# metarank/metarank

Hardware: AMD Instinct MI355X
Metric: ranked items/sec (feature assembly + 500-tree LambdaMART + ordering), Ranklens-shaped 100-item requests (higher is better)
Workload: dtype f64

## Files before the change

metarank_amd/__init__.py:

```python
from ._native import MrkError, build, lib, reload_switches
from .booster import LIGHTGBM, XGBOOST, Context, HipBooster, default_context
from .index import HipIndex
from .ranker import Batch, HipRanker, Server
from .request import Request, RequestSet
from .trending import HipTrending, TrendingBuilder
from .als import AlsBuilder
from .eval import eval_scores, evaluate, labels_from_interactions
from .train import Trainer, bin_bounds, fit_lambdamart, lambdarank_gradients
```

metarank_amd/_native.py:

```python
from __future__ import annotations

import ctypes as C
import os
import subprocess
import threading

HERE = os.path.dirname(os.path.abspath(__file__))
REPO = os.path.dirname(HERE)
CSRC = os.path.join(HERE, "csrc")
LIB_PATH = os.environ.get("MRK_LIB") or os.path.join(HERE, "libmrk_hip.so")
SOURCES = ["forest.cpp", "store.cpp", "features.cpp", "codec.cpp", "tokenizer.cpp", "weights.cpp", "capi.cpp", "capi_rank.cpp", "capi_encoder.cpp", "comm.cpp", "jit.cpp", "score.hip", "score_qs.hip", "rank.hip", "resolve.hip", "writes.hip", "encoder.hip"]
HEADERS = ["json.hpp", "forest.hpp", "runtime.hpp"]

MRK_OK = 0
ERR_INVALID_ARG, ERR_PARSE, ERR_DEVICE, ERR_DIM_MISMATCH = -1, -2, -3, -4
ERR_ARITHMETIC, ERR_UNSUPPORTED, ERR_NOT_FOUND, ERR_FEATURE_MISMATCH = -5, -6, -7, -8


class MrkError(RuntimeError):
    def __init__(self, status: int, message: str):
        super().__init__(f"[{status}] {message}")
        self.status = status
        self.message = message


def sources():
    extra = sorted(f for f in os.listdir(CSRC) if f.endswith((".cpp", ".hip")) and f not in SOURCES)
    return [os.path.join(CSRC, f) for f in SOURCES + extra]


JIT_HEADERS = ["device_types.hpp", "rank.hpp", "qs_device.hpp", "sort_device.hpp", "table_device.hpp", "walk_device.hpp", "wave_device.hpp", "rank_device.hpp"]


def embed_jit_sources() -> str:
    parts = []
    for h in JIT_HEADERS:
        lines = [ln for ln in open(os.path.join(CSRC, h)).read().split("\n")
                 if not ln.startswith("#include") and not ln.startswith("#pragma once")]
        parts.append(f"// ---- {h}\n" + "\n".join(lines))
    text = "\n".join(parts)
    assert ')MRKJIT"' not in text
    out = "\n".join('R"MRKJIT(' + p + '\n)MRKJIT"' for p in parts) + "\n"
    path = os.path.join(CSRC, "jit_embed.inc")
    if not os.path.exists(path) or open(path).read() != out:
        with open(path, "w") as f:
            f.write(out)
    return path


def write_build_id() -> str:
    import hashlib

    h = hashlib.sha256()
    for f in sorted(os.listdir(CSRC)):
        if f.endswith((".cpp", ".hip", ".hpp")):
            h.update(f.encode() + b"\0" + open(os.path.join(CSRC, f), "rb").read())
    h.update(open(os.path.join(REPO, "include", "mrk.h"), "rb").read())
    out = '"' + h.hexdigest()[:16] + '"\n'
    path = os.path.join(CSRC, "build_id.inc")
    if not os.path.exists(path) or open(path).read() != out:
        with open(path, "w") as f:
            f.write(out)
    return path


def build(force: bool = False) -> str:
    from concurrent.futures import ThreadPoolExecutor

    embed_jit_sources()
    build_id = write_build_id()
    srcs = sources()
    headers = [os.path.join(CSRC, f) for f in os.listdir(CSRC) if f.endswith((".hpp", ".inc")) and f != "build_id.inc"] + [os.path.join(REPO, "include", "mrk.h")]
    hdr_time = max(os.path.getmtime(h) for h in headers)
    hipcc = os.environ.get("HIPCC", "/opt/rocm/bin/hipcc")
    if not os.path.exists(hipcc):
        hipcc = "hipcc"
    defines = [f"-D{d}" for d in os.environ.get("MRK_DEFINES", "").split()]
    flags = ["--offload-arch=gfx950", "-O3", "-std=c++17", "-fPIC", "-Wall", "-Wno-unused-function",
             "-ffp-contract=off"] + defines
    objdir = os.environ.get("MRK_BUILD_DIR") or os.path.join(HERE, "build")
    os.makedirs(objdir, exist_ok=True)
    stamp = os.path.join(objdir, "flags.txt")
    if not os.path.exists(stamp) or open(stamp).read() != " ".join(flags):
        force = True
# ... 230 lines not shown
```

metarank_amd/csrc/capi_rank.cpp:

```cpp
#include <algorithm>
#include <atomic>
#include <chrono>
#include <condition_variable>
#include <cstring>
#include <thread>

#include <linux/futex.h>
#include <sched.h>
#include <sys/prctl.h>
#include <sys/syscall.h>
#include <time.h>
#include <unistd.h>

#include <cstdlib>

#include "features.hpp"
#include "jit.hpp"
#include "launch_shape.hpp"
#include "qs_device.hpp"
#include "rank.hpp"
#include "runtime.hpp"

namespace mrk {

void launch_prepass(mrk_ctx *ctx, const StoreDev &st, const ProgramDev &prog, const BatchDev &b, uint32_t max_req_entries, void *jit_fn);
void launch_assemble(mrk_ctx *ctx, const StoreDev &st, const ProgramDev &prog, const BatchDev &b);
void launch_sort(mrk_ctx *ctx, const BatchDev &b, int max_items);
void launch_status_or(hipStream_t stream, const int32_t *all, int world, int n_req, int32_t *status);
void launch_normalize(mrk_ctx *ctx, const BatchDev &b, int dim, int col, int mode);
void launch_normalize_big(mrk_ctx *ctx, const BatchDev &b, int dim, int col, int item_begin, int n, int *order, void *scratch);
struct SortSrc { const double *vals; const unsigned long long *raw; long long stride; int negate; };
void launch_big_sort(mrk_ctx *ctx, hipStream_t stream, const SortSrc &src, int n, int *out_order, void *scratch);
size_t big_sort_scratch_bytes(int n);
void launch_score_batch(mrk_ctx *ctx, mrk_model *m, const double *d_x, int rows, int cols, double *d_out,
                        int *d_status, const uint32_t *d_row_req);
void launch_assemble_cells(mrk_ctx *ctx, const StoreDev &st, const ProgramDev &prog, const BatchDev &b, const QsDev &q,
                           uint16_t *cells, bool f64, void *jit_fn, uint32_t max_req_entries, void *jit_rt_fn = nullptr, uint32_t thr_total = 0);
void launch_rank_fused(mrk_ctx *ctx, const StoreDev &st, const ProgramDev &prog, const BatchDev &b, uint32_t tab_entries,
                       int vals_cap, int threads, int op_split, int slices, const QsDev *q, uint16_t *cells, bool f64, void *jit_fn, size_t rt_bytes = 0);
size_t fused_lds_bytes(uint32_t tab_entries, int vals_cap, int threads, uint32_t thr_cap, size_t rt_bytes, bool split);
size_t fused_rt_max_bytes();
int fused_max_prep();
QsDev qs_device_view(const mrk_model *m);
QsForestDev qs_forest_view(const mrk_model *m);
size_t rank_one_lds_bytes(uint32_t tab_entries, int vals_cap, int threads, uint32_t thr_cap, int n_views, bool f64, size_t rt_bytes);
size_t rank_fused_score_lds_bytes(uint32_t tab_entries, int vals_cap, int threads, uint32_t thr_cap, int n_views, bool f64, size_t rt_bytes);
void launch_rank_fused_score(mrk_ctx *ctx, const StoreDev &st, const ProgramDev &prog, const BatchDev &b, uint32_t tab_entries, int vals_cap,
                             int threads, const QsDev &q, const QsForestDev &f, uint16_t *cells, bool f64, void *jit_fn);
void launch_rank_serve(mrk_ctx *ctx, hipStream_t stream, const StoreDev &st, const ProgramDev &prog, const QsDev &q, const QsForestDev &f, const ServeGangDev &gang,
                       int n_slots, int threads, size_t lds, bool f64, void *jit_fn);
void launch_rank_one(mrk_ctx *ctx, const StoreDev &st, const ProgramDev &prog, const BatchDev &b, uint32_t tab_entries, int vals_cap,
                     int threads, int op_split, const QsDev &q, const QsForestDev &f, const OneOut &out, bool f64, void *jit_fn);
void launch_rank_one_walk(mrk_ctx *ctx, const StoreDev &st, const ProgramDev &prog, const BatchDev &b, uint32_t tab_entries, int vals_cap,
                          int threads, int op_split, const WalkDev &w, const OneOut &out, bool f64, size_t lds, void *jit_fn);
void launch_rank_values(mrk_ctx *ctx, const StoreDev &st, const ProgramDev &prog, const BatchDev &b, uint32_t tab_entries, int vals_cap,
                        int threads, int op_split, const ValuesOut &out, void *jit_fn);
void launch_rank_serve_walk(mrk_ctx *ctx, hipStream_t stream, const StoreDev &st, const ProgramDev &prog, const WalkDev &w, const ServeGangDev &gang,
                            int n_slots, int threads, size_t lds, bool f64, void *jit_fn);
int load_feature_values(Store &store, const uint8_t *bytes, size_t len, int64_t now_ms);
void launch_resolve_ids(hipStream_t stream, const IdTableDev &tab, const uint8_t *d_bytes, const uint32_t *d_offs, uint32_t bytes_len, const ReqDev *d_reqs,
                        int n_req, int total, int32_t *d_item_slot, uint32_t *d_item_req, int32_t *d_load_status);

static Store &store_of(mrk_ctx *ctx) {
  if (!ctx) throw StatusError(MRK_ERR_INVALID_ARG, "null context");
  if (!ctx->store) throw StatusError(MRK_ERR_INVALID_ARG, "mrk_config_load_json must be called first");
  return *ctx->store;
}

int status_to_code(int st, std::string &msg) {
  if (st & ST_ARITHMETIC) { msg = "java.lang.ArithmeticException: / by zero (normalised rate: global `top` counter is 0)"; return MRK_ERR_ARITHMETIC; }
  if (st & ST_DIM) { msg = "dim mismatch: item embedding is shorter than the query embedding"; return MRK_ERR_DIM_MISMATCH; }
  if (st & ST_ILLEGAL_ARG) { msg = "requirement failed: Duration is limited to +-(2^63-1)ns (ca. 292 years)"; return MRK_ERR_INVALID_ARG; }
  if (st & 32) { msg = "Input data contains `inf` or a value too large, while `missing` is not set to `inf`"; return MRK_ERR_INVALID_ARG; }
  if (st & ST_BAD_IDS) { msg = "item id offsets descend or pass bytes_len (mrk_item_ids)"; return MRK_ERR_INVALID_ARG; }
  if (st & ST_TOO_MANY) { msg = "diversity over more values than the device pre-pass supports: set `top`"; return MRK_ERR_UNSUPPORTED; }
  if (st & ST_TABLE_FULL) { msg = "internal: pre-pass hash table under-sized (store changed between prepare and run?)"; return MRK_ERR_DEVICE; }
  return MRK_OK;
}

}

using namespace mrk;

struct mrk_batch {
  mrk_ctx *ctx = nullptr;
  const Program *prog = nullptr;
  int n_req = 0, total_items = 0;
  std::mutex bmu;
  DevBuf d_in, d_prep_out, d_arena, d_matrix;
  hipStream_t stream = nullptr;
  hipStream_t s() const { return stream ? stream : ctx->stream; }
  DevBuf d_out;
  size_t out_order_off = 0, out_status_off = 0, out_bytes = 0;
  PinBuf h_out;
  bool fetch_enqueued = false;
  bool direct_out = false;
  DevBuf d_cells;
  DevBuf d_sort;
  DevBuf d_norm_order;
  DevBuf d_gather;
  DevBuf d_gather_status;
  struct BigReq { int r, n_items, item_begin; };
  std::vector<BigReq> big;
  PinBuf h_in;
  HostBatch hb;
  DevBuf d_ids;
  PinBuf h_ids;
  BatchDev view{};
  std::vector<int32_t> h_status;
  std::vector<int32_t> codes;
  bool ran = false;
  bool fused_ok = false;
  uint32_t fused_entries = 0;
  int fused_vals = 1, fused_threads = 64;
  int fused_slices = 1;
  int fused_split = 1;
  bool want_matrix = false;
  bool matrix_valid = false;
  bool values = false;
  bool values_ran = false;
  bool values_direct = false;
  PinBuf h_vals;
  size_t vals_status_off = 0;
};

namespace mrk {

void free_rank_state(mrk_ctx *ctx) {
  for (int i = 0; i <= mrk_ctx::RANK_LANES_MAX; ++i) {
    void *&lane = i < mrk_ctx::RANK_LANES_MAX ? ctx->rank_lane[i] : ctx->values_lane;
    mrk_batch *b = (mrk_batch *)lane;
    if (!b) continue;
    (void)hipSetDevice(ctx->device);
    if (b->stream) {
      (void)hipStreamSynchronize(b->stream);
      (void)hipStreamDestroy(b->stream);
    }
    delete b;
    lane = nullptr;
  }
  delete ctx->registry;
  delete ctx->store;
  ctx->registry = nullptr;
  ctx->store = nullptr;
}

static size_t align_up(size_t v, size_t a) { return (v + a - 1) / a * a; }

static void quiesce_servers(mrk_ctx *ctx);

struct StoreAccess {
  mrk_ctx *ctx;
  std::shared_lock<std::shared_mutex> shared;
  std::unique_lock<std::shared_mutex> unique;
  StoreAccess(mrk_ctx *c, bool exclusive = false, bool flush = true) : ctx(c) {
    if (!ctx->store) throw StatusError(MRK_ERR_INVALID_ARG, "mrk_config_load_json must be called first");
    if (exclusive) {
      ctx->store_writers.fetch_add(1);
      unique = std::unique_lock<std::shared_mutex>(ctx->store_mu);
      ctx->store_writers.fetch_sub(1);
      if (flush) do_flush();
      return;
    }
    lock_shared();
    while (flush && ctx->store->dirty()) {
      shared.unlock();
      {
        StoreWriteLock x(ctx);
        do_flush();
// ... 208 lines not shown

static WalkDev walk_device_view(const mrk_model *m, int cols) {
  WalkDev w;
  w.image = m->d_image.as<uint8_t>();
  w.trees = m->d_trees.as<TreeRef>();
  w.chunks = m->d_chunks.as<ChunkRef>();
  w.cat_bits = m->d_cat.as<uint32_t>();
  w.n_chunks = (int32_t)m->packed.chunks.size();
  w.cols = cols;
  w.chunk_cap = (m->packed.max_chunk_bytes + 15u) & ~15u;
  w.ref_cap = ((uint32_t)m->packed.max_chunk_trees * (uint32_t)sizeof(TreeRef) + 15u) & ~15u;
  w.leaf_trees = walk_leaf_trees((int)m->packed.max_chunk_trees);
  w.pad = 0;
  w.base = m->forest.base_score;
  return w;
}
static_assert(sizeof(TreeRef) == 12 && WALK_TILE_ROWS == QS_TILE_ROWS, "launch_shape.hpp sizes the TreeRef rows and the matrix of rank_one_walk_body");

static size_t walk_one_lds_bytes(const mrk_model *m, int cols, uint32_t tab_entries, int vals_cap, int threads) {
  return rank_one_walk_lds_bytes(cols, m->forest.backend == Backend::LightGBM, m->packed.max_chunk_bytes, (int)m->packed.max_chunk_trees,
                                 walk_leaf_trees((int)m->packed.max_chunk_trees), fused_lds_bytes(tab_entries, vals_cap, threads, 0u, 0, true));
}

static bool walk_one_model(const mrk_model *model) {
  const Switches &sw = switches();
  return model && sw.rank_one_walk != 0 && (!model->qs.ok || sw.scorer_walk);
}

static bool rank_one_walk_applies(const mrk_batch &b, const mrk_model *model) {
  const Switches &sw = switches();
  if (!sw.rank_one || sw.rank_one_walk != 1 || !walk_one_model(model) || b.want_matrix || b.prog->normalises() || !b.fused_ok || b.n_req < 1 || b.n_req > sw.rank_one_max ||
      b.hb.max_items > QS_TILE_ROWS || b.view.n_overrides > 0)
    return false;
  if (b.fused_slices != 1 || b.fused_threads > 512 || b.fused_threads < b.hb.max_items) return false;
  return walk_one_lds_bytes(model, b.prog->dim, b.fused_entries, b.fused_vals, b.fused_threads) <= RANK_ONE_LDS_CAP;
}

static void run_batch(mrk_batch &b, mrk_model *model, int lo, int hi, bool sort, bool direct = false) {
  mrk_ctx *ctx = b.ctx;
  MRK_HIP(hipSetDevice(ctx->device));
  check_model_fits(model, *b.prog);
  const Switches &sw = switches();
  const int rows = hi - lo;
  const bool normalises = b.prog->normalises();
  const bool whole_matrix = normalises && (lo != 0 || hi != b.total_items);
  const bool cells = sw.rank_cells && !sw.scorer_walk && model && model->qs.ok && !b.want_matrix && rows > 0 && !normalises;
  const bool f64 = model && model->forest.backend == Backend::LightGBM;
  const bool one = direct && sort && lo == 0 && hi == b.total_items && rank_one_applies(b, model, cells);
  const bool one_walk = !one && !cells && direct && sort && rows > 0 && lo == 0 && hi == b.total_items && rank_one_walk_applies(b, model);
  const bool fused_score = !one && sort && lo == 0 && hi == b.total_items && cells && sw.rank_fused_score && b.fused_ok && b.fused_split == 1 &&
                           b.fused_slices == 1 && b.hb.max_items <= QS_TILE_ROWS && b.view.n_overrides == 0 && b.big.empty() && b.fused_threads <= 256 &&
                           rank_fused_score_lds_bytes(b.fused_entries, b.fused_vals, b.fused_threads, qs_device_view(model).thr_cap, qs_device_view(model).n_views, f64, (size_t)qs_device_view(model).rt_doubles * 8) <= 64 * 1024;
  const QsSignature *sig = cells && sw.thr_stage ? &model->qs_sig : nullptr;
  void *jit_fn = one_walk ? jit_one_walk_function(*b.prog, f64)
                 : !cells ? (b.fused_ok && model && b.fused_split == 1 && b.fused_slices == 1 ? jit_matrix_function(*b.prog) : nullptr)
                        : one ? jit_one_function(*b.prog, f64, sig)
                        : fused_score ? jit_fused_score_function(*b.prog, f64, sig)
                        : !b.fused_ok ? jit_items_function(*b.prog, f64, sig)
                        : b.fused_split > 1 || b.fused_slices > 1 ? jit_split_function(*b.prog, f64, sig) : jit_rank_function(*b.prog, f64, sig);
  void *jit_rt_fn = cells && !one && !fused_score && !b.fused_ok ? jit_items_rt_function(*b.prog, f64, sig) : nullptr;
  void *jit_prep_fn = cells && !one && !fused_score && !b.fused_ok && b.prog->prep.size() && sw.jit_prepass ? jit_prepass_function(*b.prog) : nullptr;
  LaunchOn on(ctx, b.s());
  const StoreDev st = ctx->store->device_view();
  const ProgramDev pd = b.prog->device_view();
  b.fetch_enqueued = false;
  b.direct_out = false;
  b.values_ran = b.values_direct = false;
  if (one || one_walk) {
    b.h_out.reserve(b.out_bytes);
    uint8_t *h = b.h_out.as<uint8_t>();
    const OneOut out{(double *)h, (int32_t *)(h + b.out_order_off), (int32_t *)(h + b.out_status_off),
                     (const int32_t *)(b.d_out.as<uint8_t>() + b.out_status_off) + std::max(b.n_req, 1), std::max(b.n_req, 1)};
    b.view.item_lo = 0;
    b.view.item_hi = b.total_items;
    if (one_walk)
      launch_rank_one_walk(ctx, st, pd, b.view, b.fused_entries, b.fused_vals, b.fused_threads, b.fused_split, walk_device_view(model, pd.dim), out, f64,
                           walk_one_lds_bytes(model, pd.dim, b.fused_entries, b.fused_vals, b.fused_threads), jit_fn);
    else launch_rank_one(ctx, st, pd, b.view, b.fused_entries, b.fused_vals, b.fused_threads, b.fused_split, qs_device_view(model), qs_forest_view(model), out, f64, jit_fn);
    b.matrix_valid = false;
    b.direct_out = true;
    b.ran = true;
    return;
  }
  MRK_HIP(hipMemsetAsync(b.view.status, 0, std::max<size_t>(b.n_req, 1) * 4, b.s()));
  b.view.item_lo = whole_matrix ? 0 : lo;
  b.view.item_hi = whole_matrix ? b.total_items : hi;
  if (fused_score) {
    const QsDev q = qs_device_view(model);
    b.d_cells.reserve(std::max<size_t>((size_t)b.n_req * q.n_views * QS_TILE_ROWS * 2, 16));
    launch_rank_fused_score(ctx, st, pd, b.view, b.fused_entries, b.fused_vals, b.fused_threads, q, qs_forest_view(model), b.d_cells.as<uint16_t>(), f64, jit_fn);
    b.matrix_valid = false;
    b.ran = true;
    return;
  }
  if (cells) {
    const QsDev q = qs_device_view(model);
    const size_t tile_bytes = (size_t)q.n_views * QS_TILE_ROWS * 2;
    const size_t n_tiles = ((size_t)b.total_items + QS_TILE_ROWS - 1) / QS_TILE_ROWS;
    b.d_cells.reserve(std::max<size_t>(n_tiles * tile_bytes, 16));
    if (hi % QS_TILE_ROWS && tile_bytes)
      MRK_HIP(hipMemsetAsync(b.d_cells.as<uint8_t>() + (size_t)(hi / QS_TILE_ROWS) * tile_bytes, 0, tile_bytes, b.s()));
    if (b.fused_ok) {
      launch_rank_fused(ctx, st, pd, b.view, b.fused_entries, b.fused_vals, b.fused_threads, b.fused_split, b.fused_slices, &q, b.d_cells.as<uint16_t>(), f64, jit_fn,
                        sig && sig->ok ? (size_t)sig->rt_total * 8 : 0);
    } else {
      launch_prepass(ctx, st, pd, b.view, b.fused_entries, jit_prep_fn);
      launch_assemble_cells(ctx, st, pd, b.view, q, b.d_cells.as<uint16_t>(), f64, jit_fn, b.fused_entries, jit_rt_fn, jit_rt_fn ? model->qs_sig.rt_total : 0u);
    }
    b.matrix_valid = false;
    launch_score_qs_cells(ctx, model, b.d_cells.as<uint16_t>() + (size_t)(lo / QS_TILE_ROWS) * (tile_bytes / 2), rows, b.view.scores + lo);
  } else {
    assemble_matrix(b, st, pd, jit_fn);
    b.matrix_valid = whole_matrix || (lo == 0 && hi == b.total_items);
    if (model && rows > 0) {
      launch_score_batch(ctx, model, b.view.matrix + (size_t)lo * pd.dim, rows, pd.dim, b.view.scores + lo, b.view.status, b.view.item_req + lo);
    } else if (rows > 0) {
      MRK_HIP(hipMemsetAsync(b.view.scores + lo, 0, (size_t)rows * 8, b.s()));
    }
  }
  b.view.item_lo = 0;
  b.view.item_hi = b.total_items;
  if (sort) sort_batch(b);
  b.ran = true;
}

static void run_batch(mrk_batch &b, mrk_model *model) { run_batch(b, model, 0, b.total_items, true); }

static void run_values(mrk_batch &b) {
  mrk_ctx *ctx = b.ctx;
  MRK_HIP(hipSetDevice(ctx->device));
  const Switches &sw = switches();
  const size_t T = (size_t)b.total_items, R = (size_t)std::max(b.n_req, 1);
  const bool one = sw.values_one && b.fused_ok && b.n_req >= 1 && T > 0 && b.prog->dim > 0 && b.fused_slices == 1 && b.fused_threads <= 512 &&
                   b.view.n_overrides == 0 && !b.prog->normalises() && !b.want_matrix;
  void *jit_fn = one ? jit_values_function(*b.prog) : b.fused_ok && b.fused_split == 1 && b.fused_slices == 1 ? jit_matrix_function(*b.prog) : nullptr;
  LaunchOn on(ctx, b.s());
  const StoreDev st = ctx->store->device_view();
  const ProgramDev pd = b.prog->device_view();
  b.fetch_enqueued = false;
  b.direct_out = false;
  b.values_ran = true;
  b.values_direct = false;
  b.view.item_lo = 0;
  b.view.item_hi = b.total_items;
  if (one) {
    b.vals_status_off = align_up(T * (size_t)pd.dim * 8, 256);
    b.h_vals.reserve(b.vals_status_off + 2 * R * 4);
    uint8_t *h = b.h_vals.as<uint8_t>();
    const ValuesOut out{(double *)h, (int32_t *)(h + b.vals_status_off), (const int32_t *)(b.d_out.as<uint8_t>() + b.out_status_off) + R, (int32_t)R};
    launch_rank_values(ctx, st, pd, b.view, b.fused_entries, b.fused_vals, b.fused_threads, b.fused_split, out, jit_fn);
    b.matrix_valid = false;
    b.values_direct = true;
    b.ran = true;
    return;
  }
  MRK_HIP(hipMemsetAsync(b.view.status, 0, R * 4, b.s()));
  assemble_matrix(b, st, pd, jit_fn);
// ... 304 lines not shown
      (void)st.increment_periodic(keys[i], ts_ms[i], inc[i]);
    }
  });
}
int mrk_store_increment(mrk_ctx *ctx, const char *key, int64_t inc) { STORE_PUT(increment(key, inc)); }
int mrk_store_append(mrk_ctx *ctx, const char *key, const char *value, int64_t ts_ms) { STORE_PUT(append(key, value, ts_ms)); }

int mrk_debug_fused_shape(int n_req, int max_items, int *out3) {
  const mrk::FusedShape s = mrk::fused_launch_shape(n_req, max_items);
  out3[0] = s.threads();
  out3[1] = s.split;
  out3[2] = s.slices;
  return MRK_OK;
}
int mrk_debug_scorer_split(int rows, int views, int f64, int n_cus) {
  return mrk::scorer_waves_per_tile(((long long)rows + mrk::QS_TILE_ROWS - 1) / mrk::QS_TILE_ROWS, views, f64 != 0, n_cus, mrk::QS_LEAVES, mrk::QS_TILE_ROWS);
}

int64_t mrk_debug_walk_lds(int cols, int f64, int64_t chunk_bytes, int chunk_trees, int64_t assembly_bytes, int *out_leaf_trees) {
  const int lt = mrk::walk_leaf_trees(chunk_trees);
  if (out_leaf_trees) *out_leaf_trees = lt;
  return (int64_t)mrk::rank_one_walk_lds_bytes(cols, f64 != 0, (size_t)chunk_bytes, chunk_trees, lt, (size_t)assembly_bytes);
}

int mrk_debug_clone_items(mrk_ctx *ctx, int copies, int64_t *out_items) {
  return guard([&] {
    Store &st = store_of(ctx);
    StoreWriteLock lk(ctx);
    const uint32_t n = st.clone_items(copies);
    if (out_items) *out_items = n;
  });
}

int mrk_debug_store_info(mrk_ctx *ctx, int scope, int64_t *out) {
  return guard([&] {
    Store &st = store_of(ctx);
    if (scope < 0 || scope >= SC_COUNT || !out) throw StatusError(MRK_ERR_INVALID_ARG, "bad scope");
    std::shared_lock<std::shared_mutex> lk(ctx->store_mu);
    const Table &t = st.tables[scope];
    out[0] = t.n_slots; out[1] = t.stride; out[2] = t.heap_off; out[3] = t.heap_cap;
    out[4] = (int64_t)st.tok_pool.host.size(); out[5] = (int64_t)st.f64_pool.host.size();
  });
}

int mrk_debug_batch_tables(mrk_batch *b, int64_t *out3, uint32_t *caps, int64_t n_caps) {
  return guard([&] {
    if (!b || !b->prog || !out3) throw StatusError(MRK_ERR_INVALID_ARG, "null argument");
    std::lock_guard<std::mutex> lk(b->bmu);
    const size_t n_prep = b->prog->prep.size(), n = (size_t)b->n_req * n_prep;
    out3[0] = b->fused_entries; out3[1] = b->n_req; out3[2] = (int64_t)n_prep;
    if (!caps) return;
    if (n_caps < (int64_t)n || b->hb.prep_out.size() < n) throw StatusError(MRK_ERR_INVALID_ARG, "caps is too short");
    for (size_t i = 0; i < n; ++i) caps[i] = b->hb.prep_out[i].tab_cap;
  });
}

int mrk_debug_column_distinct(mrk_ctx *ctx, const char *column, int64_t *out) {
  return guard([&] {
    Store &st = store_of(ctx);
    if (!column || !out) throw StatusError(MRK_ERR_INVALID_ARG, "null argument");
    std::shared_lock<std::shared_mutex> lk(ctx->store_mu);
    const Table &t = st.tables[SC_ITEM];
    auto it = t.col_of.find(column);
    *out = it == t.col_of.end() ? -1 : (int64_t)t.cols[(size_t)it->second].distinct;
  });
}

int mrk_store_flush(mrk_ctx *ctx) {
  return guard([&] {
    Store &st = store_of(ctx);
    StoreWriteLock lk(ctx);
    MRK_HIP(hipSetDevice(ctx->device));
    st.flush(ctx->stream);
  });
}

static const Program &program_of(mrk_ctx *ctx, const char *model_name) {
  if (!ctx || !model_name) throw StatusError(MRK_ERR_INVALID_ARG, "null argument");
  if (!ctx->registry) throw StatusError(MRK_ERR_INVALID_ARG, "mrk_config_load_json must be called first");
  const Program *p = ctx->registry->program(model_name);
  if (!p) throw StatusError(MRK_ERR_NOT_FOUND, std::string("model ") + model_name + " is not configured");
  return *p;
}

namespace {
enum : uint32_t { TK_WAITING = 0, TK_LEAD = 1, TK_DONE = 2 };
inline void futex_wait(std::atomic<uint32_t> *w, uint32_t expected) {
  (void)syscall(SYS_futex, (uint32_t *)w, FUTEX_WAIT_PRIVATE, expected, nullptr, nullptr, 0);
}
inline void futex_wake(std::atomic<uint32_t> *w) { (void)syscall(SYS_futex, (uint32_t *)w, FUTEX_WAKE_PRIVATE, 1, nullptr, nullptr, 0); }

struct RankTicket {
  mrk_model *model;
  std::string model_name;
  const mrk_request *req;
  double *scores;
  int32_t *order;
  double *matrix;
  int status = MRK_OK;
  std::string err;
  std::atomic<uint32_t> state{TK_WAITING};
  bool taken = false;
  RankTicket(mrk_model *m, const char *name, const mrk_request *r, double *s, int32_t *o, double *mat)
      : model(m), model_name(name), req(r), scores(s), order(o), matrix(mat) {}
};

// ... 1150 lines not shown
```

metarank_amd/csrc/features.cpp:

```cpp
#include "features.hpp"
#include "tzif.hpp"

#include <algorithm>
#include <cmath>
#include <cstdlib>
#include <cstring>
#include <limits>
#include <exception>
#include <set>
#include <string_view>
#include <thread>

#include "duration.hpp"
#include "encoder.hpp"
#include "jit.hpp"
#include "json.hpp"
#include "match_host.hpp"

namespace mrk {

static_assert(MATCH_MAX_QUERY == MRK_MATCH_MAX_QUERY_TOKENS && MATCH_MAX_QUERY_BM25 == MRK_MATCH_MAX_QUERY_TOKENS_BM25, "include/mrk.h names the limits");

namespace {

// ... 895 lines not shown
  return (int)std::max(1u, std::min(8u, hw ? hw : 1u));
}

template <typename Fn>
static void parallel_ranges(int64_t n, int workers, const Fn &fn) {
  if (workers <= 1 || n <= 1) { fn((int64_t)0, n, 0); return; }
  workers = (int)std::min<int64_t>(workers, n);
  std::vector<std::exception_ptr> errs((size_t)workers);
  std::vector<std::thread> th;
  th.reserve((size_t)workers - 1);
  auto run = [&](int w) {
    const int64_t lo = n * w / workers, hi = n * (w + 1) / workers;
    try { fn(lo, hi, w); } catch (...) { errs[(size_t)w] = std::current_exception(); }
  };
  for (int w = 1; w < workers; ++w) th.emplace_back(run, w);
  run(0);
  for (auto &t : th) t.join();
  for (auto &e : errs)
    if (e) std::rethrow_exception(e);
}


struct HostCell { uint8_t tag; uint64_t bits; };
HostCell host_cell(const Store &st, ScopeId scope, int32_t slot, ColRef c) {
  if (slot < 0 || c.tag < 0) return {TAG_MISSING, 0};
  const uint8_t *rec = st.record(scope, (uint32_t)slot);
  HostCell h;
  h.tag = rec[c.tag];
  memcpy(&h.bits, rec + c.val, 8);
  return h;
}

}

static bool query_text(const mrk_request &rq, const FeatureDef &f, std::string &out) {
  if (f.field.empty()) return false;
  const mrk_field *fl = fields_map_get(rq, f.field);
  if (!fl) return false;
  if (fl->type == MRK_FIELD_STRING && fl->str) { out = fl->str; return true; }
  if (fl->type == MRK_FIELD_STRING_LIST) {
    out.clear();
    for (int k = 0; k < fl->n; ++k) { if (k) out.push_back(' '); if (fl->strs && fl->strs[k]) out += fl->strs[k]; }
    return true;
  }
  return false;
}

void resolve_requests(const Program &prog, Store &store, const mrk_request *reqs, int n_req, const mrk_item_ids *ids, HostBatch &hb) {
  hb.item_slot.clear();
  hb.item_req.clear();
  hb.irf.clear();
  hb.overrides.clear();
  hb.arena_entries = hb.max_req_entries = 0;
  hb.max_doubles = hb.max_items = hb.total_items = 0;
  std::vector<int> begins((size_t)n_req + 1, 0);
  for (int r = 0; r < n_req; ++r) {
    if (reqs[r].n_items < 0 || (reqs[r].n_items > 0 && !ids && !reqs[r].item_ids)) throw StatusError(MRK_ERR_INVALID_ARG, "bad item list");
    if (reqs[r].n_items > (1 << 27)) throw StatusError(MRK_ERR_UNSUPPORTED, "requests with more than 2^27 items are not supported");
    if ((long long)begins[r] + reqs[r].n_items > INT32_MAX) throw StatusError(MRK_ERR_UNSUPPORTED, "batches of more than 2^31 items are not supported");
    begins[r + 1] = begins[r] + reqs[r].n_items;
  }
  if (ids && begins[n_req] > 0 && (!ids->bytes || !ids->offsets)) throw StatusError(MRK_ERR_INVALID_ARG, "null id bytes / offsets");
  auto id_of = [&](int r, int i) -> std::string_view {
    if (ids) {
      const uint32_t o0 = ids->offsets[begins[r] + i], o1 = ids->offsets[begins[r] + i + 1];
      if (o1 < o0 || o1 > ids->bytes_len) throw StatusError(MRK_ERR_INVALID_ARG, "mrk_item_ids: offsets descend or pass bytes_len");
      return std::string_view((const char *)ids->bytes + o0, o1 - o0);
    }
    const char *s = reqs[r].item_ids[i];
    return s ? std::string_view(s) : std::string_view("");
  };
  bool device_ids = ids != nullptr;
  if (device_ids)
    for (const HostOp &ho : prog.host_ops)
      if (ho.def->type == FType::Diversity)
        for (int r = 0; r < n_req && device_ids; ++r)
          if (std::min(ho.def->div_top, reqs[r].n_items) > PREP_MAX_VALUES) device_ids = false;
  hb.device_ids = device_ids;
  std::map<std::pair<mrk_encoder *, std::string>, std::vector<float>> queries;
  for (const HostOp &ho : prog.host_ops) {
    const FeatureDef &f = *ho.def;
    if (f.type != FType::Biencoder || !f.encoder) continue;
    std::vector<std::string> texts;
    std::string text;
    for (int r = 0; r < n_req; ++r) {
      const mrk_field *fl = fields_map_get(reqs[r], f.ext_field);
      if (fl && fl->type == MRK_FIELD_NUMBER_LIST) continue;
      if (query_text(reqs[r], f, text) && queries.emplace(std::make_pair(f.encoder, text), std::vector<float>()).second) texts.push_back(text);
    }
    if (!texts.empty()) {
      std::vector<std::vector<float>> out;
      encoder_embed_cached(f.encoder, texts, out);
      for (size_t i = 0; i < texts.size(); ++i) queries[std::make_pair(f.encoder, texts[i])] = std::move(out[i]);
    }
  }
  struct CrossValue { int req, item, dst; double v; };
  std::vector<CrossValue> cross_values;
  for (const HostOp &ho : prog.host_ops) {
    const FeatureDef &f = *ho.def;
    if (!f.cross || !f.encoder) continue;
    auto &texts = store.texts[f.name];
    const Tokenizer &tk = f.encoder->tok;
    std::vector<Encoding> rows;
    std::vector<std::pair<int, int>> where;
    std::string text;
    for (int r = 0; r < n_req; ++r) {
      if (!query_text(reqs[r], f, text)) continue;
      const std::vector<int32_t> q = tk.pieces(text);
      for (int i = 0; i < reqs[r].n_items; ++i) {
        auto it = texts.find(std::string(id_of(r, i)));
        if (it == texts.end()) continue;
        if (reqs[r].item_field_offsets && reqs[r].item_fields) {
          bool given = false;
          for (const mrk_field *p = reqs[r].item_fields + reqs[r].item_field_offsets[i], *pe = reqs[r].item_fields + reqs[r].item_field_offsets[i + 1]; p != pe; ++p)
            if (p->name && f.ext_field == p->name) { given = true; break; }
          if (given) continue;
        }
        Store::ItemText &e = it->second;
        if (!e.tokenized) { e.pieces = tk.pieces(e.text); e.tokenized = true; }
        rows.push_back(tk.assemble(q, &e.pieces));
        where.emplace_back(r, i);
      }
    }
    if (rows.empty()) continue;
    std::vector<float> logits(rows.size());
    encoder_score_rows(f.encoder, rows, logits.data());
    for (size_t k = 0; k < where.size(); ++k) cross_values.push_back({where[k].first, where[k].second, ho.dst, (double)logits[k]});
  }
  const int total = begins[n_req];
  hb.total_items = total;
  hb.reqs.resize(n_req);
  if (!device_ids) {
    hb.item_slot.resize(total);
    hb.item_req.resize(total);
  }
  hb.consts.assign((size_t)n_req * prog.n_consts, kNaN);
  hb.irf.assign((size_t)prog.n_irf * total, -1);
  hb.prep_out.assign((size_t)n_req * prog.prep.size(), PrepOut{0, 0, 0.0, 0, 0});
  for (int r = 0; r < n_req; ++r) hb.reqs[r].item_begin = begins[r];
  const uint64_t load_pct = table_load_pct();
  const int n_workers = (device_ids ? n_req >= 16384 : total >= 16384) ? host_threads() : 1;
  std::vector<const HostOp *> request_ops;
  for (const HostOp &ho : prog.host_ops) {
    const FeatureDef &f = *ho.def;
    const bool per_request = (f.type == FType::Number && f.scope == SC_RANKING) || (f.type == FType::WordCount && f.scope == SC_RANKING) ||
                             (f.type == FType::String && f.field_is_ranking) || f.type == FType::LocalTime || f.type == FType::Position ||
                             f.type == FType::ExternalRanking || f.type == FType::Biencoder || (f.type == FType::Rate && f.scope == SC_IRF) ||
                             f.type == FType::InteractedWith || f.type == FType::Diversity || f.type == FType::FieldMatch;
    if (per_request) request_ops.push_back(&ho);
  }
  const Table &item_table = store.tables[SC_ITEM];
  auto col_max_len = [&](ColRef c) -> uint64_t { return c.tag >= 0 && c.tag < (int)item_table.cols.size() ? item_table.cols[(size_t)c.tag].max_len : 0u; };
  auto vocab_bound = [&](ColRef c) -> uint64_t { return c.tag >= 0 && c.tag < (int)item_table.cols.size() ? 2ull * item_table.cols[(size_t)c.tag].distinct : 0u; };
  struct Worker { std::vector<Override> overrides; int max_items = 0, max_doubles = 0; std::vector<double> enc; };
  std::vector<Worker> workers((size_t)std::max(1, n_workers));
  std::vector<uint64_t> req_entries((size_t)n_req, 0);
  auto resolve_one = [&](int r, Worker &wk, int item_workers) {
    const mrk_request &rq = reqs[r];
    ReqDev &rd = hb.reqs[r];
    const int begin = rd.item_begin;
    std::vector<double> &enc = wk.enc;
    uint64_t arena = 0;
    rd.n_items = rq.n_items;
    wk.max_items = std::max(wk.max_items, rq.n_items);
    rd.ts_ms = rq.timestamp_ms;
    if (!device_ids) parallel_ranges(rq.n_items, rq.n_items >= 16384 ? item_workers : 1, [&](int64_t lo, int64_t hi, int) {
      const SlotMap &map = store.tables[SC_ITEM].slot_of;
      constexpr int BLOCK = 64;
      uint64_t hs[BLOCK];
      uint32_t lens[BLOCK];
      for (int64_t i0 = lo; i0 < hi; i0 += BLOCK) {
        const int nb = (int)std::min<int64_t>(BLOCK, hi - i0);
        for (int k = 0; k < nb; ++k) {
          const std::string_view id = id_of(r, (int)(i0 + k));
          lens[k] = (uint32_t)id.size();
          hs[k] = SlotMap::hash(id.data(), lens[k]);
          map.prefetch(hs[k]);
        }
        for (int k = 0; k < nb; ++k) {
          const std::string_view idv = id_of(r, (int)(i0 + k));
          const char *id = idv.data();
          const uint32_t s = map.find_hashed(hs[k], id, lens[k]);
          hb.item_slot[begin + i0 + k] = s == SlotMap::NONE ? -1 : (int32_t)s;
          hb.item_req[begin + i0 + k] = (uint32_t)r;
        }
      }
    });
    double *cs = prog.n_consts ? &hb.consts[(size_t)r * prog.n_consts] : nullptr;
    auto prefetch_record = [&](int32_t slot) {
      if (slot < 0) return;
      const Table &t = store.tables[SC_ITEM];
      const uint8_t *rec = t.rows.data() + (size_t)slot * t.stride;
      for (uint32_t o = 0; o < t.stride; o += 64) __builtin_prefetch(rec + o);
    };
    if (!prog.prep.empty() && !device_ids) {
      for (int i = 0; i < std::min(rq.n_items, 48); ++i) prefetch_record(hb.item_slot[begin + i]);
      for (const HostOp &ho : prog.host_ops) {
        if (ho.def->type != FType::InteractedWith) continue;
        const HostCell lc = host_cell(store, ho.def->scope, ho.def->scope == SC_SESSION ? rd.session_slot : rd.user_slot, prog.prep[ho.prep_base].list_col);
        if (lc.tag == TAG_MISSING) continue;
        const uint32_t off = (uint32_t)lc.bits, len = (uint32_t)(lc.bits >> 32);
        for (uint32_t k = 0; k < len; ++k) prefetch_record((int32_t)store.slot_pool.host[off + k]);
      }
    }
    for (const HostOp *hop : request_ops) {
      const HostOp &ho = *hop;
      const FeatureDef &f = *ho.def;
// ... 66 lines not shown
          const mrk_field *fl = fields_map_get(rq, f.ext_field);
          std::string_view toks[MATCH_MAX_QUERY];
          const std::string_view *q = nullptr;
          int nq = 0;
          if (fl && fl->type == MRK_FIELD_STRING_LIST) {
            if (fl->n < 0 || (fl->n > 0 && !fl->strs)) throw StatusError(MRK_ERR_INVALID_ARG, "bad string list " + f.ext_field);
            nq = fl->n;
            q = toks;
            for (int k = 0; k < nq && k < MATCH_MAX_QUERY; ++k) toks[k] = fl->strs[k] ? std::string_view(fl->strs[k]) : std::string_view("");
          }
          const int cap = f.match_method == MATCH_BM25 ? MATCH_MAX_QUERY_BM25 : MATCH_MAX_QUERY;
          const MatchPack rc = nq > cap ? MATCH_PACK_TOO_MANY
                                        : match_pack_query(f.match_method, f.termfreq.get(), q, nq, [&](std::string_view s) { return store.find_token(s); }, cs + ho.const_idx);
          if (rc == MATCH_PACK_TOO_MANY)
            throw StatusError(MRK_ERR_UNSUPPORTED, "feature " + f.name + ": " + std::to_string(nq) + " query tokens, " + std::to_string(cap) + " are supported");
          if (rc == MATCH_PACK_NOT_ASCENDING)
            throw StatusError(MRK_ERR_INVALID_ARG, "feature " + f.name + ": the query tokens are not strictly ascending in UTF-16 order (matcher.tokenize sorts and dedups)");
          break;
        }
        case FType::Rate:
          if (f.scope == SC_IRF) {
            const mrk_field *fl = fields_map_get(rq, f.scope_field);
            if (fl && fl->type == MRK_FIELD_STRING && fl->str) {
              const std::string prefix = f.scope_field + ":" + fl->str + ":";
              for (int i = 0; i < rq.n_items; ++i) {
                uint32_t s = store.slot(SC_IRF, prefix + std::string(id_of(r, i)), false);
                hb.irf[(size_t)ho.irf_id * total + begin + i] = s == Store::NO_SLOT ? -1 : (int32_t)s;
              }
            }
          }
          break;
        default: break;
      }
      if (f.type == FType::InteractedWith) {
        const ScopeId ls = f.scope;
        const int32_t vslot = ls == SC_SESSION ? rd.session_slot : rd.user_slot;
        for (size_t fi = 0; fi < f.values.size(); ++fi) {
          const PrepEntry &pe = prog.prep[ho.prep_base + fi];
          uint64_t count = 0;
          HostCell lc = host_cell(store, ls, vslot, pe.list_col);
          if (lc.tag != TAG_MISSING) {
            const uint32_t off = (uint32_t)lc.bits, len = (uint32_t)(lc.bits >> 32);
            if (device_ids) {
              count = (uint64_t)len * col_max_len(pe.item_col);
            } else {
              for (uint32_t k = 0; k < len; ++k) {
                HostCell ic = host_cell(store, SC_ITEM, (int32_t)store.slot_pool.host[off + k], pe.item_col);
                if (ic.tag == TAG_STRING_LIST) count += (uint32_t)(ic.bits >> 32);
              }
            }
          }
          PrepOut &po = hb.prep_out[(size_t)r * prog.prep.size() + ho.prep_base + fi];
          const uint32_t cap = table_capacity(std::min(count, vocab_bound(pe.item_col)), load_pct);
          po.tab_off = (uint32_t)arena;
          po.tab_cap = cap;
          arena += cap;
        }
      } else if (f.type == FType::Diversity) {
        const PrepEntry &pe = prog.prep[ho.prep_base];
        uint64_t tokens = 0;
        int taken = 0, doubles = 0;
        int mode = -1;
        if (device_ids) {
          doubles = std::min(f.div_top, rq.n_items);
          tokens = (uint64_t)doubles * col_max_len(pe.item_col);
        }
        for (int i = 0; !device_ids && i < rq.n_items && taken < f.div_top; ++i) {
          HostCell c = host_cell(store, SC_ITEM, hb.item_slot[begin + i], pe.item_col);
          if (c.tag == TAG_MISSING) continue;
          if (mode < 0) mode = (c.tag == TAG_STRING || c.tag == TAG_STRING_LIST) ? 1 : (c.tag == TAG_DOUBLE ? 2 : 0);
          if (mode == 0) break;
          if (mode == 1 && c.tag == TAG_STRING) { tokens += 1; ++taken; }
          else if (mode == 1 && c.tag == TAG_STRING_LIST) { tokens += (uint32_t)(c.bits >> 32); ++taken; }
          else if (mode == 2 && c.tag == TAG_DOUBLE) { ++doubles; ++taken; }
        }
        PrepOut &po = hb.prep_out[(size_t)r * prog.prep.size() + ho.prep_base];
        if (doubles > PREP_MAX_VALUES) {
          std::vector<double> vals;
          vals.reserve((size_t)doubles);
          int took = 0;
          for (int i = 0; i < rq.n_items && took < f.div_top; ++i) {
            HostCell c = host_cell(store, SC_ITEM, hb.item_slot[begin + i], pe.item_col);
            if (c.tag != TAG_DOUBLE) continue;
            double v;
            memcpy(&v, &c.bits, 8);
            ++took;
            if (v == v) vals.push_back(v);
          }
          std::sort(vals.begin(), vals.end(), [](double a, double b) { return a < b || (a == b && std::signbit(a) && !std::signbit(b)); });
          double med = std::numeric_limits<double>::quiet_NaN();
          const size_t m = vals.size();
          if (m == 1) med = vals[0];
          else if (m > 1) {
            const double pos = 0.5 * (double)(m + 1), fpos = std::floor(pos), dif = pos - fpos;
            const size_t ipos = (size_t)fpos;
            if (pos < 1.0) med = vals[0];
            else if (pos >= (double)m) med = vals[m - 1];
            else med = vals[ipos - 1] + dif * (vals[ipos] - vals[ipos - 1]);
          }
          po.mode = DIV_DOUBLE;
          po.scalar = med;
          po.preset = 1;
          doubles = 0;
        }
        wk.max_doubles = std::max(wk.max_doubles, doubles);
        const uint32_t cap = table_capacity(std::min(tokens, vocab_bound(pe.item_col)), load_pct);
        po.tab_off = (uint32_t)arena;
        po.tab_cap = cap;
        arena += cap;
      }
    }
    if (rq.item_field_offsets && rq.item_fields) {
      for (int i = 0; i < rq.n_items; ++i) {
        const mrk_field *fb = rq.item_fields + rq.item_field_offsets[i], *fe = rq.item_fields + rq.item_field_offsets[i + 1];
        if (fb == fe) continue;
        for (const HostOp &ho : prog.host_ops) {
          const FeatureDef &f = *ho.def;
          const uint32_t gi = (uint32_t)(begin + i);
          if (f.type == FType::Number && f.scope != SC_RANKING) {
            for (const mrk_field *p = fb; p != fe; ++p)
              if (p->type == MRK_FIELD_NUMBER && p->name && f.field == p->name) { wk.overrides.push_back({gi, (uint32_t)ho.dst, p->num}); break; }
          } else if (f.type == FType::String && !f.field_is_ranking) {
            for (const mrk_field *p = fb; p != fe; ++p) {
              if (!p->name || f.field != p->name) continue;
              if (p->type != MRK_FIELD_STRING && p->type != MRK_FIELD_STRING_LIST) continue;
              enc.assign(f.dim, 0.0);
              if (p->type == MRK_FIELD_STRING) { const char *one[1] = {p->str ? p->str : ""}; encode_string(f, one, 1, enc.data()); }
              else encode_string(f, p->strs, p->n, enc.data());
              for (int k = 0; k < f.dim; ++k) wk.overrides.push_back({gi, (uint32_t)(ho.dst + k), enc[k]});
              break;
            }
          } else if (f.type == FType::Relevancy) {
            for (const mrk_field *p = fb; p != fe; ++p)
              if (p->name && !strcmp(p->name, "relevancy")) {
                if (p->type == MRK_FIELD_NUMBER) wk.overrides.push_back({gi, (uint32_t)ho.dst, p->num});
                break;
              }
          } else if (f.type == FType::ExternalItem) {
            for (const mrk_field *p = fb; p != fe; ++p)
              if (p->name && f.ext_field == p->name) {
                if (p->type == MRK_FIELD_NUMBER && f.dim == 1) wk.overrides.push_back({gi, (uint32_t)ho.dst, p->num});
                else if (p->type == MRK_FIELD_NUMBER_LIST) {
                  if (p->n != f.dim) throw StatusError(MRK_ERR_DIM_MISMATCH, "for " + f.name + " dim mismatch: " + std::to_string(f.dim) + " != " + std::to_string(p->n));
                  for (int k = 0; k < f.dim; ++k) wk.overrides.push_back({gi, (uint32_t)(ho.dst + k), p->nums[k]});
                }
                break;
              }
          }
        }
      }
    }
    req_entries[(size_t)r] = arena;
  };
  {
    constexpr int BLOCK = 32;
    uint64_t hs[3][BLOCK];
    uint32_t lens[3][BLOCK];
    const ScopeId scs[3] = {SC_USER, SC_SESSION, SC_RANKING};
    for (int r0 = 0; r0 < n_req; r0 += BLOCK) {
      const int nb = std::min(BLOCK, n_req - r0);
      for (int k = 0; k < nb; ++k) {
        const mrk_request &rq = reqs[r0 + k];
        const char *idp[3] = {rq.user, rq.session, rq.id ? rq.id : ""};
        for (int j = 0; j < 3; ++j) {
          if (store.tables[scs[j]].slot_of.n == 0) idp[j] = nullptr;
          lens[j][k] = idp[j] ? (uint32_t)strlen(idp[j]) : 0u;
          hs[j][k] = idp[j] ? SlotMap::hash(idp[j], lens[j][k]) : 0;
          if (idp[j]) store.tables[scs[j]].slot_of.prefetch(hs[j][k]);
        }
      }
      for (int k = 0; k < nb; ++k) {
        const mrk_request &rq = reqs[r0 + k];
        const char *idp[3] = {rq.user, rq.session, rq.id ? rq.id : ""};
        int32_t out[3];
        for (int j = 0; j < 3; ++j)
          if (store.tables[scs[j]].slot_of.n == 0) idp[j] = nullptr;
        for (int j = 0; j < 3; ++j) {
          const Table &t = store.tables[scs[j]];
          const uint32_t sl = idp[j] ? t.slot_of.find_hashed(hs[j][k], idp[j], lens[j][k]) : SlotMap::NONE;
          out[j] = sl == SlotMap::NONE ? -1 : (int32_t)sl;
          if (out[j] >= 0) __builtin_prefetch(t.rows.data() + (size_t)out[j] * t.stride);
        }
        ReqDev &rd = hb.reqs[r0 + k];
        rd.user_slot = out[0];
        rd.session_slot = out[1];
        rd.ranking_slot = out[2];
      }
    }
  }
  if (n_req == 1) {
    resolve_one(0, workers[0], n_workers);
  } else {
    parallel_ranges(n_req, n_workers, [&](int64_t lo, int64_t hi, int w) {
      for (int64_t r = lo; r < hi; ++r) resolve_one((int)r, workers[(size_t)w], 1);
    });
  }
  uint64_t arena = 0;
  for (int r = 0; r < n_req; ++r) {
    if (arena + req_entries[(size_t)r] > 0xffffffffull) throw StatusError(MRK_ERR_UNSUPPORTED, "batch needs more than 2^32 hash-table entries");
    hb.reqs[r].arena_begin = (uint32_t)arena;
    for (size_t e = 0; e < prog.prep.size(); ++e) hb.prep_out[(size_t)r * prog.prep.size() + e].tab_off += (uint32_t)arena;
    hb.max_req_entries = std::max(hb.max_req_entries, req_entries[(size_t)r]);
    arena += req_entries[(size_t)r];
  }
  for (Worker &wk : workers) {
    hb.overrides.insert(hb.overrides.end(), wk.overrides.begin(), wk.overrides.end());
    hb.max_items = std::max(hb.max_items, wk.max_items);
    hb.max_doubles = std::max(hb.max_doubles, wk.max_doubles);
  }
  for (const CrossValue &c : cross_values)
    if (c.v == c.v) hb.overrides.push_back({(uint32_t)(hb.reqs[c.req].item_begin + c.item), (uint32_t)c.dst, c.v});
  hb.arena_entries = arena;
}

int debug_local_time(const char *iso, int mapper, double *out) {
  try {
    Civil c;
    if (!iso || !out || !parse_iso_datetime(iso, c)) return 0;
    *out = map_datetime(mapper, c);
    return 1;
  } catch (const StatusError &e) {
    set_last_error(e.what());
    return e.status;
  }
}

}

extern "C" {
int mrk_debug_local_time(const char *iso, int mapper, double *out) { return mrk::debug_local_time(iso, mapper, out); }
void mrk_debug_tz_reset(void) { mrk::tz_debug_reset(); }
}
```

metarank_amd/csrc/features.hpp:

```cpp
#pragma once
#include <map>
#include <memory>
#include <mutex>
#include <string>
#include <vector>

#include "rank.hpp"
#include "store.hpp"

struct mrk_encoder;

namespace mrk {

struct TermFreqDic;

enum class FType {
  Number, Boolean, WordCount, Vector, String, InteractionCount, WindowCount, Rate, InteractedWith, Diversity,
  ItemAge, LocalTime, Position, Relevancy, Biencoder, ExternalRanking, ExternalItem, FieldMatch
};

struct FeatureDef {
  FType type = FType::Number;
  std::string name;
  ScopeId scope = SC_ITEM;
// ... 34 lines not shown

enum ValueMode : int { MODE_ONLINE = 0, MODE_OFFLINE = 1 };

struct Program {
  std::string model;
  int mode = MODE_ONLINE;
  std::vector<std::string> feature_names;
  std::vector<Op> ops;
  std::vector<HostOp> host_ops;
  std::vector<PrepEntry> prep;
  std::vector<uint32_t> aux;
  int dim = 0;
  int n_consts = 0;
  int n_irf = 0;
  struct NormCol { int col; int mode; const FeatureDef *cross; };
  std::vector<NormCol> norm_cols;
  bool normalises() const {
    for (const NormCol &n : norm_cols)
      if (!n.cross || n.cross->encoder) return true;
    return false;
  }
  int item_fixed = 0;
  DevBuf d_ops, d_prep, d_aux;
  mutable std::mutex jit_mu;
  mutable void *jit = nullptr;
  mutable bool jit_failed = false;
  ProgramDev device_view() const;
  ~Program();
};

struct Registry {
  std::vector<std::unique_ptr<FeatureDef>> features;
  std::map<std::string, std::unique_ptr<Program>> programs;
  const Program *program(const std::string &model) const;
  std::unique_ptr<Program> mapping[2];
  std::map<std::string, std::unique_ptr<Program>> offline_programs;
  const Program *values_program(const char *model, int mode) const;
  ~Registry();
};

std::unique_ptr<Registry> load_config(const char *json, size_t len, Store &store, bool upload = true);
std::vector<std::string> scala_map_key_order(const std::vector<std::string> &keys);

struct HostBatch {
  std::vector<ReqDev> reqs;
  std::vector<int32_t> item_slot;
  std::vector<uint32_t> item_req;
  std::vector<double> consts;
  std::vector<int32_t> irf;
  std::vector<Override> overrides;
  std::vector<PrepOut> prep_out;
  uint64_t arena_entries = 0;
  uint64_t max_req_entries = 0;
  int max_doubles = 0;
  int max_items = 0;
  int total_items = 0;
  bool device_ids = false;
};

void resolve_requests(const Program &prog, Store &store, const mrk_request *reqs, int n_req, const mrk_item_ids *ids, HostBatch &out);

}
```

metarank_amd/csrc/jit.cpp:

```cpp
#include <hip/hip_runtime.h>
#include <hip/hiprtc.h>

#include <dlfcn.h>

#include <cstdio>
#include <cstdlib>
#include <cstring>
#include <atomic>
#include <map>
#include <memory>
#include <string>
#include <sys/stat.h>
#include <thread>
#include <unistd.h>
#include <vector>

#include "features.hpp"
#include "forest.hpp"
#include "jit.hpp"
#include "runtime.hpp"

namespace mrk {

namespace {
// ... 18 lines not shown
  for (unsigned char c : s) h = (h ^ c) * 1099511628211ull;
  return h;
}

}

std::string jit_source(const Program &prog, bool f64, int kernel, const QsSignature *sig) {
  std::string s;
  s.reserve(strlen(k_device_source) + 8192);
  for (size_t at = 0; at < switches().jit_defines.size();) {
    size_t end = switches().jit_defines.find(' ', at);
    if (end == std::string::npos) end = switches().jit_defines.size();
    std::string d = switches().jit_defines.substr(at, end - at);
    at = end + 1;
    if (d.empty()) continue;
    const size_t eq = d.find('=');
    s += "#define " + (eq == std::string::npos ? d : d.substr(0, eq) + " " + d.substr(eq + 1)) + "\n";
  }
  s += k_device_source;
  s += "\nnamespace mrk {\nnamespace {\n";
  auto table = [&](const char *name, const char *type, size_t n, const std::string &rows) {
    s += std::string("struct ") + name + " {\n  __device__ __forceinline__ constexpr " + type + " operator[](int i) const {\n    constexpr " + type +
         " t[" + std::to_string(n ? n : 1) + "] = {" + rows + "};\n    return t[i];\n  }\n};\n";
  };
  std::string rows;
  for (const Op &o : prog.ops) {
    rows += "\n      {" + std::to_string(o.kind) + "," + std::to_string(o.dst) + "," + std::to_string(o.dim) + "," + std::to_string(o.scope) + "," +
            col(o.c0) + "," + col(o.c1) + "," + col(o.c2) + "," + col(o.c3) + "," + col(o.c4) + "," + col(o.c5) + "," + std::to_string(o.i0) + "," +
            std::to_string(o.i1) + "," + std::to_string(o.i2) + "," + std::to_string(o.i3) + "," + f64_literal(o.d0) + "},";
  }
  table("JitOps", "Op", prog.ops.size(), rows);
  rows.clear();
  for (const PrepEntry &p : prog.prep)
    rows += "\n      {" + std::to_string(p.kind) + "," + col(p.item_col) + "," + std::to_string(p.list_scope) + "," + col(p.list_col) + "," +
            std::to_string(p.top) + ",0},";
  table("JitPrep", "PrepEntry", prog.prep.size(), rows);
  rows.clear();
  for (uint32_t a : prog.aux) rows += std::to_string(a) + "u,";
  table("JitAux", "uint32_t", prog.aux.size(), rows);
  s += "struct JitProg {\n  static constexpr bool is_static = true;\n";
  s += "  static constexpr int32_t n_ops = " + std::to_string(prog.ops.size()) + ", n_prep = " + std::to_string(prog.prep.size()) +
       ", dim = " + std::to_string(prog.dim) + ", n_consts = " + std::to_string(prog.n_consts) + ", item_fixed = " + std::to_string(switches().jit_record_regs ? prog.item_fixed : 0) + ";\n";
  s += "  JitOps ops;\n  JitPrep prep;\n  JitAux aux;\n};\n";
  std::string qs = "mrk::QsDyn";
  if (sig && sig->ok && kernel != JIT_MATRIX && kernel != JIT_PREPASS && kernel != JIT_ONE_WALK && kernel != JIT_SERVE_WALK && kernel != JIT_VALUES) {
    table("JitSigRows", "QsSig", sig->cols.size(), sig->text);
    s += "struct JitQs {\n  static constexpr bool is_static = true;\n  static constexpr int n_feats = " + std::to_string(sig->cols.size()) +
         ", n_views = " + std::to_string(sig->n_views) + ";\n  static constexpr uint32_t thr_cap = " + std::to_string(sig->thr_cap) +
         "u, thr_total = " + std::to_string(sig->thr_total) + "u, rt_total = " + std::to_string(sig->rt_total) +
         "u;\n  __device__ __forceinline__ constexpr QsSig operator[](int i) const { return JitSigRows{}[i]; }\n};\n";
    qs = "mrk::JitQs";
  }
  s += "}  // namespace\n}  // namespace mrk\n\n";
  std::string attr;
  {
    const int w = switches().jit_waves >= 1 && switches().jit_waves <= 8 ? switches().jit_waves : 4;
    attr = " __attribute__((amdgpu_waves_per_eu(" + std::to_string(w) + ", " + std::to_string(w) + ")))";
  }
  const std::string b64 = f64 ? "true" : "false";
  if (kernel == JIT_ALL || kernel == JIT_RANK)
    s += "extern \"C\" __global__ void __launch_bounds__(256)" + attr + "\nmrk_jit_rank_cells"
         "(mrk::StoreDev st, mrk::BatchDev b, uint32_t tab_entries, int vals_cap, mrk::QsDev q, uint16_t *cells, int mode) {\n"
         "  mrk::rank_fused_cells_body<" + b64 + ", false, " + qs + ">(st, mrk::JitProg{}, b, tab_entries, vals_cap, q, cells, mode);\n}\n";
  if (kernel == JIT_ALL || kernel == JIT_SPLIT)
    s += "extern \"C\" __global__ void __launch_bounds__(512)" + attr + "\nmrk_jit_rank_cells_split"
         "(mrk::StoreDev st, mrk::BatchDev b, uint32_t tab_entries, int vals_cap, mrk::QsDev q, uint16_t *cells, int mode) {\n"
         "  mrk::rank_fused_cells_body<" + b64 + ", true, " + qs + ">(st, mrk::JitProg{}, b, tab_entries, vals_cap, q, cells, mode);\n}\n";
  if ((kernel == JIT_ALL && f64) || kernel == JIT_MATRIX)
    s += "extern \"C\" __global__ void __launch_bounds__(256)" + attr + "\nmrk_jit_rank_matrix"
         "(mrk::StoreDev st, mrk::BatchDev b, uint32_t tab_entries, int vals_cap, int mode) {\n"
         "  mrk::rank_fused_matrix_body<false>(st, mrk::JitProg{}, b, tab_entries, vals_cap, mode);\n}\n";
  if (kernel == JIT_VALUES)
    s += "extern \"C\" __global__ void __launch_bounds__(512) __attribute__((amdgpu_waves_per_eu(2, 2)))\nmrk_jit_rank_values"
         "(mrk::StoreDev st, mrk::BatchDev b, uint32_t tab_entries, int vals_cap, int mode, mrk::ValuesOut out) {\n"
         "  mrk::rank_values_body<true>(st, mrk::JitProg{}, b, tab_entries, vals_cap, mode, out);\n}\n";
  if (kernel == JIT_ALL || kernel == JIT_ITEMS)
    s += "extern \"C\" __global__ void __launch_bounds__(256)" + attr + "\nmrk_jit_assemble_cells"
         "(mrk::StoreDev st, mrk::BatchDev b, mrk::QsDev q, uint16_t *cells, uint32_t lds_entries) {\n"
         "  mrk::assemble_cells_body<" + b64 + ", " + qs + ">(st, mrk::JitProg{}, b, q, cells, lds_entries);\n}\n";
  if ((kernel == JIT_ALL || kernel == JIT_ITEMS_RT) && qs != "mrk::QsDyn" && jit_items_rt_applies(sig))
    s += "extern \"C\" __global__ void __launch_bounds__(512)" + attr + "\nmrk_jit_assemble_cells_rt"
         "(mrk::StoreDev st, mrk::BatchDev b, mrk::QsDev q, uint16_t *cells, uint32_t lds_entries) {\n"
         "  mrk::assemble_cells_rt_body<" + b64 + ", " + qs + ">(st, mrk::JitProg{}, b, q, cells, lds_entries);\n}\n";
  if (kernel == JIT_ALL || kernel == JIT_ONE)
    s += "extern \"C\" __global__ void __launch_bounds__(512) __attribute__((amdgpu_waves_per_eu(2, 2)))\nmrk_jit_rank_one"
         "(mrk::StoreDev st, mrk::BatchDev b, uint32_t tab_entries, int vals_cap, mrk::QsDev q, mrk::QsForestDev f, int mode, mrk::OneOut out) {\n"
         "  mrk::rank_one_body<" + b64 + ", " + qs + ">(st, mrk::JitProg{}, b, tab_entries, vals_cap, q, f, mode, out);\n}\n";
  if (kernel == JIT_ALL || kernel == JIT_FUSED_SCORE)
    s += "extern \"C\" __global__ void __launch_bounds__(256)" + attr + "\nmrk_jit_rank_fused_score"
         "(mrk::StoreDev st, mrk::BatchDev b, uint32_t tab_entries, int vals_cap, mrk::QsDev q, mrk::QsForestDev f, uint16_t *cells) {\n"
         "  mrk::rank_fused_score_body<" + b64 + ", " + qs + ">(st, mrk::JitProg{}, b, tab_entries, vals_cap, q, f, cells);\n}\n";
  if ((kernel == JIT_ALL && f64) || kernel == JIT_PREPASS)
    s += "extern \"C\" __global__ void __launch_bounds__(256)\nmrk_jit_prepass"
         "(mrk::StoreDev st, mrk::BatchDev b, uint32_t lds_entries) {\n"
         "  mrk::prepass_body(st, mrk::JitProg{}, b, lds_entries);\n}\n";
  if (kernel == JIT_ALL || kernel == JIT_SERVE)
    s += "extern \"C\" __global__ void __launch_bounds__(512) __attribute__((amdgpu_waves_per_eu(2, 2)))\nmrk_jit_rank_serve"
         "(mrk::StoreDev st, mrk::QsDev q, mrk::QsForestDev f, mrk::ServeGangDev gang) {\n"
         "  mrk::rank_serve_body<" + b64 + ", " + qs + ">(st, mrk::JitProg{}, q, f, gang);\n}\n";
  if (kernel == JIT_ALL || kernel == JIT_ONE_WALK)
    s += "extern \"C\" __global__ void __launch_bounds__(512) __attribute__((amdgpu_waves_per_eu(2, 2)))\nmrk_jit_rank_one_walk"
         "(mrk::StoreDev st, mrk::BatchDev b, uint32_t tab_entries, int vals_cap, mrk::WalkDev w, int mode, mrk::OneOut out) {\n"
         "  mrk::rank_one_walk_body<" + b64 + ">(st, mrk::JitProg{}, b, tab_entries, vals_cap, w, mode, out);\n}\n";
  if (kernel == JIT_ALL || kernel == JIT_SERVE_WALK)
    s += "extern \"C\" __global__ void __launch_bounds__(512) __attribute__((amdgpu_waves_per_eu(2, 2)))\nmrk_jit_rank_serve_walk"
         "(mrk::StoreDev st, mrk::WalkDev w, mrk::ServeGangDev gang) {\n"
         "  mrk::rank_serve_walk_body<" + b64 + ">(st, mrk::JitProg{}, w, gang);\n}\n";
  return s;
}

std::vector<char> jit_compile(const std::string &source, std::string &log) {
  hiprtcProgram p = nullptr;
  if (hiprtcCreateProgram(&p, source.c_str(), "mrk_rank_jit.hip", 0, nullptr, nullptr) != HIPRTC_SUCCESS)
    throw StatusError(MRK_ERR_DEVICE, "hiprtcCreateProgram failed");
// ... 307 lines not shown
```

metarank_amd/csrc/rank.hip:

```cpp
#include <hip/hip_runtime.h>

#include <cstdint>
#include <mutex>
#include <utility>

#include "rank_device.hpp"
#include "sort_device.hpp"
#include "runtime.hpp"

namespace mrk {

namespace {

__global__ void __launch_bounds__(PREP_THREADS)
prepass_kernel(StoreDev st, ProgramDev prog, BatchDev b, uint32_t lds_entries) { prepass_body(st, prog, b, lds_entries); }

__global__ void __launch_bounds__(ASM_THREADS)
assemble_kernel(StoreDev st, ProgramDev prog, BatchDev b) {
  const int gi0 = b.item_lo + blockIdx.x * ASM_THREADS + threadIdx.x;
  const bool active = gi0 < b.item_hi;
  if (!__any(active)) return;
  const int gi = active ? gi0 : b.item_hi - 1;
  const int r = (int)b.item_req[gi];
  const ReqDev rq = b.reqs[r];
// ... 221 lines not shown
  }
}

static void launch_override_cells(mrk_ctx *ctx, const BatchDev &b, const QsDev &q, uint16_t *cells, bool f64) {
  if (b.n_overrides <= 0) return;
  ScopedKernelTimer timer(ctx, "override");
  const dim3 grid((b.n_overrides + 255) / 256);
  if (f64) hipLaunchKernelGGL(override_cells_kernel<true>, grid, dim3(256), 0, ctx->launch, b, q, cells);
  else hipLaunchKernelGGL(override_cells_kernel<false>, grid, dim3(256), 0, ctx->launch, b, q, cells);
  MRK_HIP(hipGetLastError());
}

void launch_assemble_cells(mrk_ctx *ctx, const StoreDev &st, const ProgramDev &prog, const BatchDev &b, const QsDev &q,
                           uint16_t *cells, bool f64, void *jit_fn, uint32_t max_req_entries, void *jit_rt_fn, uint32_t thr_total) {
  if (b.item_hi <= b.item_lo) return;
  if (jit_rt_fn) {
    ScopedKernelTimer timer(ctx, "assemble");
    const int n_items = b.item_hi - b.item_lo;
    constexpr uint32_t RT_LDS_TABLE_BYTES = 24 * 1024;
    uint32_t lds_entries = switches().items_lds && prog.n_prep > 0 && (uint64_t)max_req_entries * 8 <= RT_LDS_TABLE_BYTES ? max_req_entries : 0u;
    const size_t lds = (size_t)thr_total * 8 + (size_t)lds_entries * 8;
    int threads = (long long)n_items >= 2ll * 512 * ctx->n_cus ? 512 : 256;
    if (switches().items_rt_threads == 256 || switches().items_rt_threads == 512) threads = switches().items_rt_threads;
    const int n_blocks = (n_items + threads - 1) / threads;
    const int per_cu = std::max(1, std::min((int)((160 * 1024) / std::max<size_t>(lds, 1)), 16 / (threads / 64)));
    const unsigned grid = (unsigned)std::min(n_blocks, per_cu * ctx->n_cus);
    StoreDev a_st = st;
    BatchDev a_b = b;
    QsDev a_q = q;
    void *args[] = {&a_st, &a_b, &a_q, &cells, &lds_entries};
    MRK_HIP(hipModuleLaunchKernel((hipFunction_t)jit_rt_fn, grid, 1, 1, (unsigned)threads, 1, 1, (unsigned)lds, ctx->launch, args, nullptr));
    launch_override_cells(ctx, b, q, cells, f64);
    return;
  }
  {
    ScopedKernelTimer timer(ctx, "assemble");
    const dim3 grid((b.item_hi - b.item_lo + ASM_THREADS - 1) / ASM_THREADS);
    constexpr uint32_t ITEMS_LDS_TABLE_BYTES = 24 * 1024;
    uint32_t lds_entries = switches().items_lds && prog.n_prep > 0 && (uint64_t)max_req_entries * 8 <= ITEMS_LDS_TABLE_BYTES ? max_req_entries : 0u;
    const size_t lds = (size_t)lds_entries * 8;
    if (jit_fn) {
      StoreDev a_st = st;
      BatchDev a_b = b;
      QsDev a_q = q;
      void *args[] = {&a_st, &a_b, &a_q, &cells, &lds_entries};
      MRK_HIP(hipModuleLaunchKernel((hipFunction_t)jit_fn, grid.x, 1, 1, ASM_THREADS, 1, 1, (unsigned)lds, ctx->launch, args, nullptr));
    } else if (f64) hipLaunchKernelGGL(assemble_cells_kernel<true>, grid, dim3(ASM_THREADS), lds, ctx->launch, st, prog, b, q, cells, lds_entries);
    else hipLaunchKernelGGL(assemble_cells_kernel<false>, grid, dim3(ASM_THREADS), lds, ctx->launch, st, prog, b, q, cells, lds_entries);
    MRK_HIP(hipGetLastError());
  }
  launch_override_cells(ctx, b, q, cells, f64);
}

size_t fused_lds_bytes(uint32_t tab_entries, int vals_cap, int threads, uint32_t thr_cap, size_t rt_bytes, bool split) {
  const size_t staging = (size_t)((threads + 63) / 64) * 2 * thr_cap * 8;
  return (size_t)tab_entries * 8 + (size_t)vals_cap * 8 + FUSED_MAX_PREP * sizeof(PrepOut) + PREP_INTS * sizeof(int) +
         16 + std::max(staging, rt_bytes <= (split ? FUSED_RT_MAX_BYTES_SPLIT : FUSED_RT_MAX_BYTES) ? rt_bytes : 0);
}
size_t fused_rt_max_bytes() { return FUSED_RT_MAX_BYTES_SPLIT; }
int fused_max_prep() { return FUSED_MAX_PREP; }

void launch_rank_fused(mrk_ctx *ctx, const StoreDev &st, const ProgramDev &prog, const BatchDev &b, uint32_t tab_entries,
                       int vals_cap, int threads, int op_split, int slices, const QsDev *q, uint16_t *cells, bool f64, void *jit_fn, size_t rt_bytes) {
  if (b.n_req <= 0) return;
  int mode = (op_split > 1 ? op_split : 1) | ((slices > 1 ? slices : 1) << 8);
  const unsigned grid = (unsigned)b.n_req * (unsigned)(slices > 1 ? slices : 1);
  size_t lds = fused_lds_bytes(tab_entries, vals_cap, threads, q ? q->thr_cap : 0u, q && cells ? rt_bytes : 0, op_split > 1 || slices > 1);
  if (switches().fused_lds_min > 0) lds = std::max(lds, (size_t)switches().fused_lds_min);
  {
    ScopedKernelTimer timer(ctx, "assemble");
    if (!jit_fn) lds_optin(ctx, !cells ? (const void *)rank_fused_matrix_kernel : f64 ? (const void *)rank_fused_cells_kernel<true> : (const void *)rank_fused_cells_kernel<false>);
    if (!cells && jit_fn) {
      StoreDev a_st = st;
      BatchDev a_b = b;
      int a_vals = vals_cap;
      void *args[] = {&a_st, &a_b, &tab_entries, &a_vals, &mode};
      MRK_HIP(hipModuleLaunchKernel((hipFunction_t)jit_fn, grid, 1, 1, (unsigned)threads, 1, 1, (unsigned)lds, ctx->launch, args, nullptr));
    } else if (cells && jit_fn) {
      StoreDev a_st = st;
      BatchDev a_b = b;
      QsDev a_q = *q;
      int a_vals = vals_cap;
      void *args[] = {&a_st, &a_b, &tab_entries, &a_vals, &a_q, &cells, &mode};
      MRK_HIP(hipModuleLaunchKernel((hipFunction_t)jit_fn, grid, 1, 1, (unsigned)threads, 1, 1, (unsigned)lds, ctx->launch, args, nullptr));
    } else if (!cells) hipLaunchKernelGGL(rank_fused_matrix_kernel, dim3(grid), dim3(threads), lds, ctx->launch, st, prog, b, tab_entries, vals_cap, mode);
    else if (f64) hipLaunchKernelGGL(rank_fused_cells_kernel<true>, dim3(grid), dim3(threads), lds, ctx->launch, st, prog, b, tab_entries, vals_cap, *q, cells, mode);
    else hipLaunchKernelGGL(rank_fused_cells_kernel<false>, dim3(grid), dim3(threads), lds, ctx->launch, st, prog, b, tab_entries, vals_cap, *q, cells, mode);
    MRK_HIP(hipGetLastError());
  }
  if (!cells) {
    if (b.n_overrides > 0) {
      ScopedKernelTimer timer(ctx, "override");
      hipLaunchKernelGGL(override_kernel, dim3((b.n_overrides + 255) / 256), dim3(256), 0, ctx->launch, b, prog.dim);
      MRK_HIP(hipGetLastError());
    }
  } else {
    launch_override_cells(ctx, b, *q, cells, f64);
  }
}

size_t rank_values_lds_bytes(uint32_t tab_entries, int vals_cap, int threads) { return 16 + fused_lds_bytes(tab_entries, vals_cap, threads, 0u, 0, true); }

void launch_rank_values(mrk_ctx *ctx, const StoreDev &st, const ProgramDev &prog, const BatchDev &b, uint32_t tab_entries, int vals_cap,
                        int threads, int op_split, const ValuesOut &out, void *jit_fn) {
  if (b.n_req <= 0) return;
  int mode = op_split > 1 ? op_split : 1;
  const size_t lds = rank_values_lds_bytes(tab_entries, vals_cap, threads);
  ScopedKernelTimer timer(ctx, "rank_values");
  if (jit_fn) {
    StoreDev a_st = st;
    BatchDev a_b = b;
    ValuesOut a_out = out;
    int a_vals = vals_cap;
    void *args[] = {&a_st, &a_b, &tab_entries, &a_vals, &mode, &a_out};
    MRK_HIP(hipModuleLaunchKernel((hipFunction_t)jit_fn, (unsigned)b.n_req, 1, 1, (unsigned)threads, 1, 1, (unsigned)lds, ctx->launch, args, nullptr));
  } else {
    lds_optin(ctx, (const void *)rank_values_kernel);
    hipLaunchKernelGGL(rank_values_kernel, dim3(b.n_req), dim3(threads), lds, ctx->launch, st, prog, b, tab_entries, vals_cap, mode, out);
    MRK_HIP(hipGetLastError());
  }
}

__global__ void __launch_bounds__(SORT_THREADS)
norm_position_apply_kernel(const int *__restrict__ order, int n, double *colp, int dim) {
  const int s = blockIdx.x * SORT_THREADS + threadIdx.x;
  if (s >= n) return;
  double *p = colp + (size_t)order[s] * dim;
  const double v = *p;
  if (v == v) *p = __ddiv_rn((double)s, (double)n);
}

void launch_normalize_big(mrk_ctx *ctx, const BatchDev &b, int dim, int col, int item_begin, int n, int *order, void *scratch) {
  ScopedKernelTimer timer(ctx, "normalize");
  double *colp = b.matrix + (size_t)item_begin * dim + col;
  const SortSrc src{colp, nullptr, dim, 0};
  launch_big_sort(ctx, ctx->launch, src, n, order, scratch);
  hipLaunchKernelGGL(norm_position_apply_kernel, dim3((n + SORT_THREADS - 1) / SORT_THREADS), dim3(SORT_THREADS), 0, ctx->launch, order, n, colp, dim);
  MRK_HIP(hipGetLastError());
}

size_t rank_one_lds_bytes(uint32_t tab_entries, int vals_cap, int threads, uint32_t thr_cap, int n_views, bool f64, size_t rt_bytes) {
  const size_t nw = (size_t)threads / 64;
  const size_t scoring = 8 * nw * (QS_LEAVES * (f64 ? 8 : 4) + QS_TILE_ROWS) + QS_TILE_ROWS * 8;
  return (size_t)n_views * QS_TILE_ROWS * 2 + 16 + std::max(fused_lds_bytes(tab_entries, vals_cap, threads, thr_cap, rt_bytes, true), scoring);
}

void launch_rank_one(mrk_ctx *ctx, const StoreDev &st, const ProgramDev &prog, const BatchDev &b, uint32_t tab_entries, int vals_cap,
                     int threads, int op_split, const QsDev &q, const QsForestDev &f, const OneOut &out, bool f64, void *jit_fn) {
  if (b.n_req <= 0) return;
  int mode = op_split > 1 ? op_split : 1;
  const size_t lds = rank_one_lds_bytes(tab_entries, vals_cap, threads, q.thr_cap, f.n_views, f64, (size_t)q.rt_doubles * 8);
// ... 132 lines not shown
```

metarank_amd/csrc/rank_device.hpp:

```cpp
#pragma once
#include <hip/hip_runtime.h>

#include "qs_device.hpp"
#include "rank.hpp"
#include "sort_device.hpp"
#include "table_device.hpp"
#include "walk_device.hpp"
#include "wave_device.hpp"

#ifdef MRK_PHASE_CLOCKS
__device__ unsigned long long mrk_phase_clocks[64];
#define MRK_PHASE(prev, acc)                                                   \
  do {                                                                         \
    const unsigned long long t_ = clock64();                                   \
    (acc) += t_ - (prev);                                                      \
    (prev) = t_;                                                               \
  } while (0)
#else
#define MRK_PHASE(prev, acc) do { } while (0)
#endif

namespace mrk {

namespace {

__device__ __forceinline__ double d_nan() { return __longlong_as_double(0x7ff8000000000000LL); }

struct Cell {
  uint32_t tag;
  uint64_t bits;
  __device__ __forceinline__ double f64() const { return __longlong_as_double((long long)bits); }
  __device__ __forceinline__ long long i64() const { return (long long)bits; }
  __device__ __forceinline__ uint32_t lo() const { return (uint32_t)bits; }
  __device__ __forceinline__ uint32_t hi() const { return (uint32_t)(bits >> 32); }
};

__device__ __forceinline__ const uint8_t *record(const StoreDev &st, int scope, int slot) {
  if (slot < 0) return nullptr;
  return st.tab[scope].rows + (size_t)slot * st.tab[scope].stride;
}

__device__ __forceinline__ Cell load_cell(const uint8_t *rec, ColRef c, int idx = 0) {
  Cell out;
  if (rec == nullptr || c.tag < 0) {
    out.tag = TAG_MISSING;
    out.bits = 0;
    return out;
  }
  out.tag = rec[c.tag];
  out.bits = *(const uint64_t *)(rec + c.val + idx * 8);
  return out;
}

__device__ __forceinline__ const uint32_t *list_tokens(const StoreDev &st, const uint8_t *rec, uint32_t off) {
  return (off & LIST_INLINE_BIT) ? (const uint32_t *)(rec + (off & ~LIST_INLINE_BIT)) : st.tok_pool + off;
}

__device__ __forceinline__ double list_f64(const StoreDev &st, uint32_t off, uint32_t k) {
  return (off & LIST_F32_BIT) ? (double)st.f32_pool[(off & ~LIST_F32_BIT) + k] : st.f64_pool[off + k];
// ... 88 lines not shown
    if (mine && !isn)
      for (int j = 0; j < n_raw; ++j) {
        const double w = s_vals[j];
        rank += (w < v || (w == v && j < tid)) ? 1 : 0;
      }
    __syncthreads();
    if (mine && !isn) s_vals[rank] = v;
    __syncthreads();
  } else {
    for (int i = tid; i < n_raw; i += nthr) {
      double v = s_vals[i];
      if (v != v) { s_vals[i] = __longlong_as_double(0x7ff0000000000000LL); atomicAdd(&s_misc[1], 1); }
    }
    int p2 = 1;
    while (p2 < n_raw) p2 <<= 1;
    for (int i = n_raw + tid; i < p2; i += nthr) s_vals[i] = __longlong_as_double(0x7ff0000000000000LL);
    __syncthreads();
    for (int k = 2; k <= p2; k <<= 1) {
      for (int j = k >> 1; j > 0; j >>= 1) {
        for (int i = tid; i < p2; i += nthr) {
          const int ixj = i ^ j;
          if (ixj > i) {
            const double a = s_vals[i], c2 = s_vals[ixj];
            const bool up = (i & k) == 0;
            if ((a > c2) == up) { s_vals[i] = c2; s_vals[ixj] = a; }
          }
        }
        __syncthreads();
      }
    }
  }
  const int m = n_raw - s_misc[1];
  if (m <= 0) return d_nan();
  const double pos = 0.5 * (double)(m + 1);
  const double fpos = floor(pos);
  const int ipos = (int)fpos;
  const double dif = pos - fpos;
  if (pos < 1.0) return s_vals[0];
  if (pos >= (double)m) return s_vals[m - 1];
  const double lower = s_vals[ipos - 1], upper = s_vals[ipos];
  return __dadd_rn(lower, __dmul_rn(dif, __dsub_rn(upper, lower)));
}



template <typename Prog>
__device__ __forceinline__ bool prepass_waves_ok(const Prog &prog) {
  bool ok = true;
  for (int e = 0; e < prog.n_prep; ++e)
    if (prog.prep[e].kind == PREP_DIVERSITY && prog.prep[e].top > 64) ok = false;
  return ok;
}

template <typename Prog>
__device__ __forceinline__ void prepass_interacted_with(const StoreDev &st, const Prog &prog, const BatchDev &b, int r, const ReqDev &rq,
                                                        unsigned long long *tab_base, uint32_t tab_sub, PrepOut *po_out, int lane_id, int n_lanes) {
  const int n_prep = prog.n_prep;
  for (int e0 = 0; e0 < n_prep;) {
    const PrepEntry pe0 = prog.prep[e0];
    if (pe0.kind != PREP_IW_FIELD) { ++e0; continue; }
    int n = 1;
    while (n < PREP_GROUP && e0 + n < n_prep) {
      const PrepEntry q = prog.prep[e0 + n];
      if (q.kind != PREP_IW_FIELD || q.list_scope != pe0.list_scope || q.list_col.tag != pe0.list_col.tag || q.list_col.val != pe0.list_col.val) break;
      ++n;
    }
    ColRef col[PREP_GROUP];
    unsigned long long *tab[PREP_GROUP];
    uint32_t cap[PREP_GROUP];
#pragma unroll
    for (int u = 0; u < PREP_GROUP; ++u) {
      const int e = e0 + (u < n ? u : 0);
      col[u] = prog.prep[e].item_col;
      tab[u] = tab_base + (po_out[e].tab_off - tab_sub);
      cap[u] = po_out[e].tab_cap;
    }
    const int vslot = pe0.list_scope == SC_SESSION ? rq.session_slot : rq.user_slot;
    const Cell lc = load_cell(record(st, pe0.list_scope, vslot), pe0.list_col);
    if (lc.tag != TAG_MISSING) {
      const uint32_t off = lc.lo(), len = lc.hi();
      for (uint32_t k = (uint32_t)lane_id; k < len; k += (uint32_t)n_lanes) {
        const uint8_t *irec = record(st, SC_ITEM, (int)st.slot_pool[off + k]);
        Cell ic[PREP_GROUP];
#pragma unroll
        for (int u = 0; u < PREP_GROUP; ++u) {
          ic[u].tag = TAG_MISSING;
          ic[u].bits = 0;
          if (u < n) ic[u] = load_cell(irec, col[u]);
        }
#pragma unroll
        for (int u = 0; u < PREP_GROUP; ++u) {
          if (u < n) {
            const bool list = ic[u].tag == TAG_STRING_LIST;
            if (table_add_list(list_tokens(st, irec, ic[u].lo()), tab[u], cap[u], list ? ic[u].hi() : 0u)) atomicOr(&b.status[r], ST_TABLE_FULL);
          }
        }
      }
    }
    e0 += n;
  }


}

template <typename Prog>
__device__ __forceinline__ void prepass_diversity_wave(const StoreDev &st, const Prog &prog, const BatchDev &b, int r, const ReqDev &rq,
                                                       unsigned long long *tab_base, uint32_t tab_sub, PrepOut *po_out, const PrepScratch &sc) {
  const int lane = threadIdx.x & 63;
  const int n_prep = prog.n_prep;
  int *s_first = sc.first();
  int *s_tokens = sc.tokens();
#ifdef MRK_PHASE_CLOCKS
  unsigned long long dv_t = clock64(), dv_acc[3] = {0, 0, 0};
#endif
  for (int e0 = 0; e0 < n_prep;) {
    if (prog.prep[e0].kind != PREP_DIVERSITY || po_out[e0].preset) { ++e0; continue; }
    int ent[DIV_GROUP];
    int n = 0, e1 = e0;
    for (; e1 < n_prep && n < DIV_GROUP; ++e1) {
      if (prog.prep[e1].kind != PREP_DIVERSITY || po_out[e1].preset) continue;
#pragma unroll
      for (int u = 0; u < DIV_GROUP; ++u) if (u == n) ent[u] = e1;
      ++n;
    }
    ColRef col[DIV_GROUP];
    unsigned long long *tab[DIV_GROUP];
    uint32_t cap[DIV_GROUP];
    int top[DIV_GROUP];
#pragma unroll
    for (int u = 0; u < DIV_GROUP; ++u) {
      if (u >= n) ent[u] = e0;
      col[u] = prog.prep[ent[u]].item_col;
      top[u] = prog.prep[ent[u]].top;
      tab[u] = tab_base + (po_out[ent[u]].tab_off - tab_sub);
      cap[u] = po_out[ent[u]].tab_cap;
    }
    const uint8_t *keep_rec = nullptr;
    Cell keep[DIV_GROUP];
#pragma unroll
    for (int u = 0; u < DIV_GROUP; ++u) { keep[u].tag = TAG_MISSING; keep[u].bits = 0; }
    for (int base = 0; base < rq.n_items; base += 64) {
      const int i = base + lane;
      if (i < rq.n_items) {
        const uint8_t *irec = record(st, SC_ITEM, b.item_slot[rq.item_begin + i]);
        Cell c[DIV_GROUP];
#pragma unroll
        for (int u = 0; u < DIV_GROUP; ++u) {
          c[u].tag = TAG_MISSING;
          c[u].bits = 0;
          if (u < n) c[u] = load_cell(irec, col[u]);
        }
#pragma unroll
        for (int u = 0; u < DIV_GROUP; ++u) {
          if (u < n && c[u].tag != TAG_MISSING) atomicMin(&s_first[ent[u]], (i << 8) | (int)c[u].tag);
          if (base == 0) keep[u] = c[u];
        }
        if (base == 0) keep_rec = irec;
      }
      wave_lds_sync();
      bool all = true;
#pragma unroll
      for (int u = 0; u < DIV_GROUP; ++u) all = all && (u >= n || s_first[ent[u]] != 0x7fffffff);
      wave_lds_sync();
      if (all) break;
    }
    int mode[DIV_GROUP];
#pragma unroll
    for (int u = 0; u < DIV_GROUP; ++u) {
      const int first = u < n ? s_first[ent[u]] : 0x7fffffff;
      const int htag = first != 0x7fffffff ? (first & 255) : (int)TAG_MISSING;
      mode[u] = (htag == TAG_STRING || htag == TAG_STRING_LIST) ? DIV_STRING : (htag == TAG_DOUBLE ? DIV_DOUBLE : DIV_EMPTY);
    }
    MRK_PHASE(dv_t, dv_acc[0]);
    bool any_string = false;
#pragma unroll
    for (int u = 0; u < DIV_GROUP; ++u) any_string = any_string || (u < n && mode[u] == DIV_STRING);
    if (lane < DIV_GROUP) s_tokens[lane] = 0;
    wave_lds_sync();
    if (any_string) {
      int running[DIV_GROUP];
#pragma unroll
      for (int u = 0; u < DIV_GROUP; ++u) running[u] = 0;
      for (int base = 0; base < rq.n_items; base += 64) {
        bool more = false;
#pragma unroll
        for (int u = 0; u < DIV_GROUP; ++u) more = more || (u < n && mode[u] == DIV_STRING && running[u] < top[u]);
        if (!more) break;
        const int i = base + lane;
        Cell c[DIV_GROUP];
        bool cand[DIV_GROUP];
        const uint8_t *irec = base == 0 ? keep_rec : (i < rq.n_items ? record(st, SC_ITEM, b.item_slot[rq.item_begin + i]) : nullptr);
#pragma unroll
        for (int u = 0; u < DIV_GROUP; ++u) {
          c[u].tag = TAG_MISSING;
          c[u].bits = 0;
          if (u < n && mode[u] == DIV_STRING) c[u] = base == 0 ? keep[u] : load_cell(irec, col[u]);
          cand[u] = c[u].tag == TAG_STRING || c[u].tag == TAG_STRING_LIST;
        }
#pragma unroll
        for (int u = 0; u < DIV_GROUP; ++u) {
          int total = 0;
          const int excl = wave_scan_flag(u < n && cand[u], total);
          if (u < n && mode[u] == DIV_STRING) {
            const bool take = cand[u] && running[u] + excl < top[u];
            const bool one = take && c[u].tag == TAG_STRING;
            const uint32_t tlen = take && !one ? c[u].hi() : 0u;
            uint32_t failed = table_add(tab[u], cap[u], c[u].lo(), one) ? 0u : 1u;
            failed += table_add_list(list_tokens(st, irec, c[u].lo()), tab[u], cap[u], tlen);
            if (failed) atomicOr(&b.status[r], ST_TABLE_FULL);
            if (take) atomicAdd(&s_tokens[u], one ? 1 : (int)tlen);
          }
          running[u] += total;
        }
      }
      wave_lds_sync();
    }
    if (lane == 0) {
#pragma unroll
      for (int u = 0; u < DIV_GROUP; ++u)
        if (u < n && mode[u] != DIV_DOUBLE) {
          po_out[ent[u]].mode = mode[u];
          po_out[ent[u]].scalar = mode[u] == DIV_STRING ? (double)s_tokens[u] : 0.0;
        }
    }
    wave_lds_sync();
    MRK_PHASE(dv_t, dv_acc[1]);
#pragma unroll
    for (int u = 0; u < DIV_GROUP; ++u) {
      if (u >= n || mode[u] != DIV_DOUBLE) continue;
      int running = 0;
      for (int base = 0; base < rq.n_items && running < top[u]; base += 64) {
        const int i = base + lane;
        Cell c;
        c.tag = TAG_MISSING;
        c.bits = 0;
        if (base == 0) c = keep[u];
        else if (i < rq.n_items) c = load_cell(record(st, SC_ITEM, b.item_slot[rq.item_begin + i]), col[u]);
        const bool cand = c.tag == TAG_DOUBLE;
        int total;
        const int rank = running + wave_scan_flag(cand, total);
        if (cand && rank < top[u]) {
          if (rank < sc.vals_cap) sc.vals[rank] = c.f64();
          else atomicOr(&b.status[r], ST_TOO_MANY);
        }
        running += total;
      }
      wave_lds_sync();
      const double scalar = wave_median_of(sc.vals, min(min(running, top[u]), min(sc.vals_cap, 64)));
      if (lane == 0) {
        po_out[ent[u]].mode = DIV_DOUBLE;
        po_out[ent[u]].scalar = scalar;
      }
      wave_lds_sync();
    }
    MRK_PHASE(dv_t, dv_acc[2]);
    e0 = e1;
  }
#ifdef MRK_PHASE_CLOCKS
  if (threadIdx.x == 0)
    for (int i = 0; i < 3; ++i) atomicAdd(&mrk_phase_clocks[8 + i], dv_acc[i]);
#endif
}

template <typename Prog>
__device__ __forceinline__ void prepass_request(const StoreDev &st, const Prog &prog, const BatchDev &b, int r, const ReqDev &rq,
                                unsigned long long *tab_base, uint32_t tab_sub, PrepOut *po_out, const PrepScratch &sc) {
  const int tid = threadIdx.x;
  const int nthr = blockDim.x;
  const int n_prep = prog.n_prep;
  int *s_first = sc.first();
  int *s_misc = sc.misc();
  int *s_tokens = sc.tokens();

  {
    uint32_t lo = 0xffffffffu, hi = 0;
    for (int e = 0; e < n_prep; ++e) {
      const uint32_t o = po_out[e].tab_off - tab_sub;
      lo = min(lo, o);
      hi = max(hi, o + po_out[e].tab_cap);
    }
    for (uint32_t i = lo + tid; i < hi; i += nthr) tab_base[i] = 0ull;
    for (int e = tid; e < n_prep; e += nthr) s_first[e] = 0x7fffffff;
  }
  __syncthreads();
  MRK_PHASE(sc.clk, sc.acc[0]);
  if (prepass_waves_ok(prog)) {
    const bool lone = nthr <= 64;
    const int wave = tid >> 6;
    if (lone || wave != 0) prepass_interacted_with(st, prog, b, r, rq, tab_base, tab_sub, po_out, lone ? tid : tid - 64, lone ? nthr : nthr - 64);
    if (wave == 0) prepass_diversity_wave(st, prog, b, r, rq, tab_base, tab_sub, po_out, sc);
#ifdef MRK_PHASE_CLOCKS
    if (tid == 64) atomicAdd(&mrk_phase_clocks[2], clock64() - sc.clk);
    if (tid == 0) atomicAdd(&mrk_phase_clocks[3], clock64() - sc.clk);
#endif
    __syncthreads();
    MRK_PHASE(sc.clk, sc.acc[1]);
    return;
  }


  for (int e0 = 0; e0 < n_prep;) {
    const PrepEntry pe0 = prog.prep[e0];
    if (pe0.kind != PREP_IW_FIELD) { ++e0; continue; }
    int n = 1;
    while (n < PREP_GROUP && e0 + n < n_prep) {
      const PrepEntry q = prog.prep[e0 + n];
      if (q.kind != PREP_IW_FIELD || q.list_scope != pe0.list_scope || q.list_col.tag != pe0.list_col.tag || q.list_col.val != pe0.list_col.val) break;
      ++n;
    }
    ColRef col[PREP_GROUP];
    unsigned long long *tab[PREP_GROUP];
    uint32_t cap[PREP_GROUP];
#pragma unroll
    for (int u = 0; u < PREP_GROUP; ++u) {
      const int e = e0 + (u < n ? u : 0);
      col[u] = prog.prep[e].item_col;
      tab[u] = tab_base + (po_out[e].tab_off - tab_sub);
      cap[u] = po_out[e].tab_cap;
    }
    const int vslot = pe0.list_scope == SC_SESSION ? rq.session_slot : rq.user_slot;
    const Cell lc = load_cell(record(st, pe0.list_scope, vslot), pe0.list_col);
    if (lc.tag != TAG_MISSING) {
      const uint32_t off = lc.lo(), len = lc.hi();
      for (uint32_t k = tid; k < len; k += nthr) {
        const uint8_t *irec = record(st, SC_ITEM, (int)st.slot_pool[off + k]);
        Cell ic[PREP_GROUP];
#pragma unroll
        for (int u = 0; u < PREP_GROUP; ++u) {
          ic[u].tag = TAG_MISSING;
          ic[u].bits = 0;
          if (u < n) ic[u] = load_cell(irec, col[u]);
        }
#pragma unroll
        for (int u = 0; u < PREP_GROUP; ++u) {
          if (u < n) {
            const bool list = ic[u].tag == TAG_STRING_LIST;
            if (table_add_list(list_tokens(st, irec, ic[u].lo()), tab[u], cap[u], list ? ic[u].hi() : 0u)) atomicOr(&b.status[r], ST_TABLE_FULL);
          }
        }
      }
    }
    e0 += n;
  }

  MRK_PHASE(sc.clk, sc.acc[1]);
  for (int e0 = 0; e0 < n_prep;) {
    if (prog.prep[e0].kind != PREP_DIVERSITY || po_out[e0].preset) { ++e0; continue; }
    int ent[PREP_GROUP];
    int n = 0, e1 = e0;
    for (; e1 < n_prep && n < PREP_GROUP; ++e1) {
      if (prog.prep[e1].kind != PREP_DIVERSITY || po_out[e1].preset) continue;
#pragma unroll
      for (int u = 0; u < PREP_GROUP; ++u) if (u == n) ent[u] = e1;
      ++n;
    }
    ColRef col[PREP_GROUP];
    unsigned long long *tab[PREP_GROUP];
    uint32_t cap[PREP_GROUP];
    int top[PREP_GROUP];
#pragma unroll
    for (int u = 0; u < PREP_GROUP; ++u) {
      if (u >= n) ent[u] = e0;
      col[u] = prog.prep[ent[u]].item_col;
      top[u] = prog.prep[ent[u]].top;
      tab[u] = tab_base + (po_out[ent[u]].tab_off - tab_sub);
      cap[u] = po_out[ent[u]].tab_cap;
    }
    const bool single = rq.n_items <= nthr;
    const uint8_t *keep_rec = nullptr;
    Cell keep[PREP_GROUP];
#pragma unroll
    for (int u = 0; u < PREP_GROUP; ++u) { keep[u].tag = TAG_MISSING; keep[u].bits = 0; }
    for (int base = 0; base < rq.n_items; base += nthr) {
      const int i = base + tid;
      if (i < rq.n_items) {
        const uint8_t *irec = record(st, SC_ITEM, b.item_slot[rq.item_begin + i]);
        Cell c[PREP_GROUP];
#pragma unroll
        for (int u = 0; u < PREP_GROUP; ++u) {
          c[u].tag = TAG_MISSING;
          c[u].bits = 0;
          if (u < n) c[u] = load_cell(irec, col[u]);
        }
#pragma unroll
        for (int u = 0; u < PREP_GROUP; ++u) {
          if (u < n && c[u].tag != TAG_MISSING) atomicMin(&s_first[ent[u]], (i << 8) | (int)c[u].tag);
          if (single) keep[u] = c[u];
        }
        if (single) keep_rec = irec;
      }
      __syncthreads();
      bool all = true;
#pragma unroll
      for (int u = 0; u < PREP_GROUP; ++u) all = all && (u >= n || s_first[ent[u]] != 0x7fffffff);
      __syncthreads();
      if (all) break;
    }
    int mode[PREP_GROUP];
#pragma unroll
    for (int u = 0; u < PREP_GROUP; ++u) {
      const int first = u < n ? s_first[ent[u]] : 0x7fffffff;
      const int htag = first != 0x7fffffff ? (first & 255) : (int)TAG_MISSING;
      mode[u] = (htag == TAG_STRING || htag == TAG_STRING_LIST) ? DIV_STRING : (htag == TAG_DOUBLE ? DIV_DOUBLE : DIV_EMPTY);
    }
    MRK_PHASE(sc.clk, sc.acc[2]);
    bool any_string = false;
#pragma unroll
    for (int u = 0; u < PREP_GROUP; ++u) any_string = any_string || (u < n && mode[u] == DIV_STRING);
    if (tid < PREP_GROUP) s_tokens[tid] = 0;
    __syncthreads();
    if (any_string) {
      int running[PREP_GROUP];
#pragma unroll
      for (int u = 0; u < PREP_GROUP; ++u) running[u] = 0;
      for (int base = 0; base < rq.n_items; base += nthr) {
        bool more = false;
#pragma unroll
        for (int u = 0; u < PREP_GROUP; ++u) more = more || (u < n && mode[u] == DIV_STRING && running[u] < top[u]);
        if (!more) break;
        const int i = base + tid;
        Cell c[PREP_GROUP];
        bool cand[PREP_GROUP];
        const uint8_t *irec = single ? keep_rec : (i < rq.n_items ? record(st, SC_ITEM, b.item_slot[rq.item_begin + i]) : nullptr);
#pragma unroll
        for (int u = 0; u < PREP_GROUP; ++u) {
          c[u].tag = TAG_MISSING;
          c[u].bits = 0;
          if (u < n && mode[u] == DIV_STRING) c[u] = single ? keep[u] : load_cell(irec, col[u]);
          cand[u] = c[u].tag == TAG_STRING || c[u].tag == TAG_STRING_LIST;
        }
        int excl[PREP_GROUP], total[PREP_GROUP];
        block_scan_flags(cand, n, sc.wave_tot(), excl, total);
#pragma unroll
        for (int u = 0; u < PREP_GROUP; ++u) {
          if (u < n && mode[u] == DIV_STRING) {
            const bool take = cand[u] && running[u] + excl[u] < top[u];
            const bool one = take && c[u].tag == TAG_STRING;
            const uint32_t tlen = take && !one ? c[u].hi() : 0u;
            uint32_t failed = table_add(tab[u], cap[u], c[u].lo(), one) ? 0u : 1u;
            failed += table_add_list(list_tokens(st, irec, c[u].lo()), tab[u], cap[u], tlen);
            if (failed) atomicOr(&b.status[r], ST_TABLE_FULL);
            if (take) atomicAdd(&s_tokens[u], one ? 1 : (int)tlen);
          }
          running[u] += total[u];
        }
      }
      __syncthreads();
    }
    if (tid == 0) {
#pragma unroll
      for (int u = 0; u < PREP_GROUP; ++u)
        if (u < n && mode[u] != DIV_DOUBLE) {
          po_out[ent[u]].mode = mode[u];
          po_out[ent[u]].scalar = mode[u] == DIV_STRING ? (double)s_tokens[u] : 0.0;
        }
    }
    MRK_PHASE(sc.clk, sc.acc[3]);
#pragma unroll
    for (int u = 0; u < PREP_GROUP; ++u) {
      if (u >= n || mode[u] != DIV_DOUBLE) continue;
      if (tid == 0) { s_misc[0] = 0; s_misc[1] = 0; }
      __syncthreads();
      int running = 0;
      for (int base = 0; base < rq.n_items && running < top[u]; base += nthr) {
        const int i = base + tid;
        Cell c;
        c.tag = TAG_MISSING;
        c.bits = 0;
        if (single) c = keep[u];
        else if (i < rq.n_items) c = load_cell(record(st, SC_ITEM, b.item_slot[rq.item_begin + i]), col[u]);
        const bool cand = c.tag == TAG_DOUBLE;
        int total;
        const int rank = running + block_scan_flag(cand, sc.wave_tot(), total);
        if (cand && rank < top[u]) {
          if (rank < sc.vals_cap) sc.vals[rank] = c.f64();
          else atomicOr(&b.status[r], ST_TOO_MANY);
        }
        running += total;
      }
      __syncthreads();
      const double scalar = median_of(sc.vals, min(min(running, top[u]), sc.vals_cap), s_misc);
      if (tid == 0) {
        po_out[ent[u]].mode = DIV_DOUBLE;
        po_out[ent[u]].scalar = scalar;
      }
      __syncthreads();
    }
    MRK_PHASE(sc.clk, sc.acc[4]);
    e0 = e1;
  }
  __syncthreads();
}
// ... 441 lines not shown
    case OP_STRING_INDEX: return 1;
    default: return 0;
  }
}
#ifndef MRK_PRE_GROUP_BUDGET
#define MRK_PRE_GROUP_BUDGET 48
#endif
constexpr int PRE_GROUP_BUDGET = MRK_PRE_GROUP_BUDGET;
template <typename Prog, bool IN_REGS>
__device__ __forceinline__ constexpr int op_group_end(int lo) {
  int w = 0, hi = lo;
  while (hi < Prog::n_ops) {
    const Op op = Prog{}.ops[hi];
    const int wi = op_pre_weight(op) + (op_has_primary(op) && !(IN_REGS && op_primary_in_item(op)) ? 3 : 0);
    if (hi > lo && w + wi > PRE_GROUP_BUDGET) break;
    w += wi;
    ++hi;
  }
  return hi;
}
constexpr int OP_SPLIT_MAX = 4;
__device__ __forceinline__ constexpr int op_cost(const Op &op) {
  switch (op.kind) {
    case OP_INTERACTED: return 5 * op.dim;
    case OP_DIVERSITY: return 7;
    case OP_RATE: return (op.i0 == RATE_ITEM ? 3 : 6) * op.dim;
    case OP_BIENCODER: return 40;
    case OP_FIELD_MATCH: return 12;
    default: return op.dim > 0 ? op.dim : 1;
  }
}
template <typename Prog>
__device__ __forceinline__ constexpr int op_owner(int oi) {
  int load[OP_SPLIT_MAX] = {0, 0, 0, 0};
  int owner = 0;
  for (int k = 0; k <= oi && k < Prog::n_ops; ++k) {
    owner = 0;
    for (int g = 1; g < OP_SPLIT_MAX; ++g)
      if (load[g] < load[owner]) owner = g;
    load[owner] += op_cost(Prog{}.ops[k]);
  }
  return owner;
}

template <typename Prog, bool IN_REGS, int LO, typename F>
__device__ __forceinline__ void run_groups(F &&f) {
  if constexpr (LO < Prog::n_ops) {
    constexpr int HI = op_group_end<Prog, IN_REGS>(LO);
    f(IntC<LO>{}, IntC<HI>{});
    run_groups<Prog, IN_REGS, HI>(f);
  }
}

template <bool SPLIT, typename Prog, typename Sink, typename IR>
__device__ __forceinline__ void assemble_item_rec(const StoreDev &st, const Prog &prog, const BatchDev &b, int gi, int r,
                                                  const ReqDev &rq, const unsigned long long *tab_base, uint32_t tab_sub,
                                                  const PrepOut *pos, const Sink &sink, int islot, const IR &ir, int og, int G_arg) {
  const int G = SPLIT ? G_arg : 1;
  const uint8_t *irec = ir.p;
  const double NaN = d_nan();

  auto other_record = [&](const Op &op) -> const uint8_t * {
    if (op.kind == OP_ITEM_AGE) return nullptr;
    return record(st, op.scope, scoped_slot(rq, op.scope, islot));
  };
  auto primary_cell = [&](const Op &op) -> Cell {
    Cell pc;
    pc.tag = TAG_MISSING;
    pc.bits = 0;
    if (!op_has_primary(op)) return pc;
    return op_primary_in_item(op) ? rec_cell(ir, op.c0) : load_cell(other_record(op), op.c0);
  };
  auto primary_list_record = [&](const Op &op) -> const uint8_t * { return op_primary_in_item(op) ? irec : other_record(op); };

  auto prefetch_op = [&](const Op &op, const Cell &pc, OpPre &pre) __attribute__((always_inline)) {
    switch (op.kind) {
      case OP_VECTOR: {
        const bool has = pc.tag == TAG_DOUBLE_LIST;
#pragma unroll
        for (int k = 0; k < PRE_F64; ++k) {
          pre.d[k] = 0.0;
          if (k < op.dim && has && (uint32_t)k < pc.hi()) pre.d[k] = list_f64(st, pc.lo(), (uint32_t)k);
        }
        break;
      }
      case OP_STRING_INDEX: {
        pre.tok[0] = 0u;
        if (pc.tag == TAG_STRING_LIST && pc.hi() > 0) pre.tok[0] = list_tokens(st, primary_list_record(op), pc.lo())[0];
        break;
      }
      case OP_DIVERSITY: case OP_FIELD_MATCH: {
        const uint32_t len = pc.tag == TAG_STRING_LIST ? pc.hi() : 0u;
        const uint32_t *toks = list_tokens(st, irec, pc.lo());
#pragma unroll
        for (int t = 0; t < TOK_BATCH; ++t) pre.tok[t] = (uint32_t)t < len ? toks[t] : 0u;
        break;
      }
      case OP_INTERACTED: {
#pragma unroll
        for (int u = 0; u < IW_BATCH; ++u) {
          pre.fc[u].tag = TAG_MISSING;
          pre.fc[u].bits = 0;
          if (u < op.dim) {
            ColRef col;
            col.tag = (int32_t)prog.aux[op.i0 + 2 * u];
            col.val = (int32_t)prog.aux[op.i0 + 2 * u + 1];
            pre.fc[u] = rec_cell(ir, col);
          }
        }
// ... 175 lines not shown
            double v = NaN;
            if (valid && !thrown) {
              if (!norm) {
                v = (double)tv[u] / (double)bv[u];
              } else if (gtv[u] == 0) {
                if (sink.active) atomicOr(&b.status[r], ST_ARITHMETIC);
                thrown = true;
              } else {
                const double ratio = long_div_to_double(gbv[u], gtv[u]);
                const double num = __dadd_rn(op.d0, (double)tv[u]);
                const double den = __dadd_rn(__dmul_rn(op.d0, ratio), (double)bv[u]);
                v = num / den;
              }
            }
            sink.put(dst + k0 + u, v);
          }
        }
        break;
      }
      case OP_INTERACTED: {
        for (int f0 = 0; f0 < op.dim; f0 += IW_BATCH) {
          Cell fc[IW_BATCH];
          uint32_t tk[IW_BATCH][IW_TOK];
#pragma unroll
          for (int u = 0; u < IW_BATCH; ++u) {
            fc[u] = pre.fc[u];
#pragma unroll
            for (int t = 0; t < IW_TOK; ++t) tk[u][t] = pre.tok[u * IW_TOK + t];
          }
          if (f0 > 0) {
#pragma unroll
            for (int u = 0; u < IW_BATCH; ++u) {
              fc[u].tag = TAG_MISSING;
              fc[u].bits = 0;
              if (f0 + u < op.dim) {
                ColRef col;
                col.tag = (int32_t)prog.aux[op.i0 + 2 * (f0 + u)];
                col.val = (int32_t)prog.aux[op.i0 + 2 * (f0 + u) + 1];
                fc[u] = rec_cell(ir, col);
              }
            }
#pragma unroll
            for (int u = 0; u < IW_BATCH; ++u) {
              const uint32_t len = fc[u].tag == TAG_STRING_LIST ? fc[u].hi() : 0u;
              const uint32_t *toks = list_tokens(st, irec, fc[u].lo());
#pragma unroll
              for (int t = 0; t < IW_TOK; ++t) tk[u][t] = (uint32_t)t < len ? toks[t] : 0u;
            }
          }
#pragma unroll
          for (int u = 0; u < IW_BATCH; ++u) {
            if (f0 + u >= op.dim) break;
            const PrepOut po = pos[op.i1 + f0 + u];
            const unsigned long long *tab = tab_base + (po.tab_off - tab_sub);
            const uint32_t len = fc[u].tag == TAG_STRING_LIST ? fc[u].hi() : 0u;
            double cnt = table_sum_tokens<IW_TOK>(tab, po.tab_cap, tk[u], len, 0.0);
            if (wave_any(len > (uint32_t)IW_TOK))
              cnt = table_sum_list(list_tokens(st, irec, fc[u].lo()) + IW_TOK, tab, po.tab_cap, len > (uint32_t)IW_TOK ? len - IW_TOK : 0u, cnt);
            sink.put(dst + f0 + u, cnt);
          }
        }
        break;
      }
      case OP_DIVERSITY: {
        const PrepOut po = pos[op.i1];
        const Cell c = pc;
        double v = NaN;
        if (po.mode == DIV_EMPTY) {
          v = 0.0;
        } else if (po.mode == DIV_DOUBLE) {
          if (c.tag == TAG_DOUBLE) v = c.f64() - po.scalar;
        } else {
          const unsigned long long *tab = tab_base + (po.tab_off - tab_sub);
          const bool one = c.tag == TAG_STRING, list = c.tag == TAG_STRING_LIST;
          const double w1 = 0.0 + (double)table_get(tab, po.tab_cap, c.lo(), one);
          const uint32_t len = list ? c.hi() : 0u;
          uint32_t dtk[TOK_BATCH];
#pragma unroll
          for (int t = 0; t < TOK_BATCH; ++t) dtk[t] = pre.tok[t];
          double wl = table_sum_tokens<TOK_BATCH>(tab, po.tab_cap, dtk, len, 0.0);
          if (wave_any(len > (uint32_t)TOK_BATCH))
            wl = table_sum_list(list_tokens(st, irec, c.lo()) + TOK_BATCH, tab, po.tab_cap, len > (uint32_t)TOK_BATCH ? len - TOK_BATCH : 0u, wl);
          if (one || list) v = (one ? w1 : wl) / po.scalar;
        }
        sink.put(dst + 0, v);
        break;
      }
      case OP_ITEM_AGE: {
        const Cell c = pc;
        double v = NaN;
        if (c.tag == TAG_DOUBLE) {
          const long long updated = java_round(c.f64() * 1000.0);
          long long diff = (long long)((unsigned long long)rq.ts_ms - (unsigned long long)updated);
          if (diff < 0) diff = (long long)(0ull - (unsigned long long)diff);
          if (diff < 0 || diff > 9223372036854LL) { if (sink.active) atomicOr(&b.status[r], ST_ILLEGAL_ARG); }
          else v = (double)(diff / 1000);
        }
        sink.put(dst + 0, v);
        break;
      }
      case OP_CONST: {
        const double *cs = b.consts + (size_t)r * prog.n_consts + op.i0;
        for (int k = 0; k < op.dim; ++k) sink.put(dst + k, cs[k]);
        break;
      }
      case OP_FILL_NAN: {
        for (int k = 0; k < op.dim; ++k) sink.put(dst + k, NaN);
        break;
      }
      case OP_BIENCODER: {
        const double *cs = b.consts + (size_t)r * prog.n_consts + op.i0;
        const int qn = (int)cs[0];
        const Cell c = pc;
        double v = NaN;
        if (qn >= 0 && c.tag == TAG_DOUBLE_LIST) {
          if ((int)c.hi() < qn) {
            if (sink.active) atomicOr(&b.status[r], ST_DIM);
          } else {
            double top = 0.0, a = 0.0, bs = 0.0;
            auto step = [&](int k, double x) {
              const float q = (float)cs[1 + k];
              top = __dadd_rn(top, __dmul_rn((double)q, x));
              a = __dadd_rn(a, (double)__fmul_rn(q, q));
              bs = __dadd_rn(bs, __dmul_rn(x, x));
            };
            if (c.lo() & LIST_F32_BIT) {
              const float *item = st.f32_pool + (c.lo() & ~LIST_F32_BIT);
              int k = 0;
// ... 36 lines not shown
  sink.begin();
  if constexpr (prog_is_static<Prog>(0)) {
    Cell pc[Prog::n_ops > 0 ? Prog::n_ops : 1];
    OpPre pre[Prog::n_ops > 0 ? Prog::n_ops : 1];
#ifdef MRK_PHASE_CLOCKS
    unsigned long long t_op = clock64(), op_acc[Prog::n_ops > 0 ? Prog::n_ops : 1] = {}, pre_acc = 0;
#endif
    constexpr bool in_regs = IR::in_regs;
    run_groups<Prog, in_regs, 0>([&](auto lo_c, auto hi_c) __attribute__((always_inline)) {
      constexpr int lo = decltype(lo_c)::value, hi = decltype(hi_c)::value;
      static_for<lo, hi>([&](auto ic) __attribute__((always_inline)) {
        constexpr int oi = decltype(ic)::value;
        constexpr Op op = Prog{}.ops[oi];
        constexpr int own = op_owner<Prog>(oi);
        if (G == 1 || (own & (G - 1)) == og) pc[oi] = primary_cell(op);
      });
      static_for<lo, hi>([&](auto ic) __attribute__((always_inline)) {
        constexpr int oi = decltype(ic)::value;
        constexpr Op op = Prog{}.ops[oi];
        constexpr int own = op_owner<Prog>(oi);
        if (G == 1 || (own & (G - 1)) == og) prefetch_op(op, pc[oi], pre[oi]);
      });
      MRK_PHASE(t_op, pre_acc);
      static_for<lo, hi>([&](auto ic) __attribute__((always_inline)) {
        constexpr int oi = decltype(ic)::value;
        constexpr Op op = Prog{}.ops[oi];
        constexpr int own = op_owner<Prog>(oi);
        if (G == 1 || (own & (G - 1)) == og) run_op(op, pc[oi], pre[oi]);
        MRK_PHASE(t_op, op_acc[oi]);
      });
    });
#ifdef MRK_PHASE_CLOCKS
    if (threadIdx.x == 0)
      for (int i = 0; i < Prog::n_ops && i < 48; ++i) atomicAdd(&mrk_phase_clocks[16 + i], op_acc[i]);
    if (threadIdx.x == 0) atomicAdd(&mrk_phase_clocks[7], pre_acc);
#endif
  } else {
    for (int oi = 0; oi < prog.n_ops; ++oi) {
      if (G > 1 && (oi & (G - 1)) != og) continue;
      const Op op = prog.ops[oi];
      const Cell pc = primary_cell(op);
      OpPre pre;
      prefetch_op(op, pc, pre);
      run_op(op, pc, pre);
    }
  }
  sink.finish();
}

template <typename P> __device__ __forceinline__ constexpr auto prog_item_pieces(int) -> decltype(P::item_fixed) { return (P::item_fixed + 15) / 16; }
template <typename P> __device__ __forceinline__ constexpr int prog_item_pieces(...) { return 0; }
constexpr int REC_MAX_PIECES = 24;

template <bool SPLIT = false, typename Prog, typename Sink>
__device__ __forceinline__ void assemble_item(const StoreDev &st, const Prog &prog, const BatchDev &b, int gi, int r,
                                              const ReqDev &rq, const unsigned long long *tab_base, uint32_t tab_sub,
                                              const PrepOut *pos, const Sink &sink, int og = 0, int G = 1) {
  const int islot = sink.active ? b.item_slot[gi] : -1;
  const uint8_t *irec = record(st, SC_ITEM, islot);
  constexpr int NP = prog_item_pieces<Prog>(0);
  if constexpr (NP > 0 && NP <= REC_MAX_PIECES) {
    const RegRec<NP> ir = load_record_regs<NP>(irec);
    assemble_item_rec<SPLIT>(st, prog, b, gi, r, rq, tab_base, tab_sub, pos, sink, islot, ir, og, G);
  } else {
    const PtrRec ir{irec};
    assemble_item_rec<SPLIT>(st, prog, b, gi, r, rq, tab_base, tab_sub, pos, sink, islot, ir, og, G);
  }
}


template <bool SPLIT, typename Prog, typename SinkMaker>
__device__ __forceinline__ void rank_fused_body(const StoreDev &st, const Prog &prog, const BatchDev &b, uint32_t tab_entries,
                                                int vals_cap, uint32_t thr_cap, int mode, const SinkMaker &make_sink, uint32_t lds_skip = 0,
                                                const double *rt_src = nullptr, uint32_t rt_doubles = 0, int blk = -1) {
  const int op_split = SPLIT ? ((mode & 255) > 1 ? (mode & 255) : 1) : 1;
  const int slices = SPLIT ? (((mode >> 8) & 255) > 1 ? ((mode >> 8) & 255) : 1) : 1;
  extern __shared__ __align__(16) uint8_t smem_base[];
  uint8_t *smem = smem_base + lds_skip;
  unsigned long long *s_tab = (unsigned long long *)smem;
  double *s_vals = (double *)(smem + (size_t)tab_entries * 8);
  PrepOut *s_po = (PrepOut *)(smem + (size_t)tab_entries * 8 + (size_t)vals_cap * 8);
  int *s_int = (int *)(s_po + FUSED_MAX_PREP);
  const size_t thr_at = ((size_t)((uint8_t *)(s_int + PREP_INTS) - smem) + 15) & ~(size_t)15;
  qs_lds_double *s_thr_all = (qs_lds_double *)(smem + thr_at);
  qs_lds_double *s_thr = s_thr_all + (size_t)(threadIdx.x >> 6) * 2 * thr_cap;
  const int bid = blk < 0 ? (int)blockIdx.x : blk;
  const int r = bid / slices, sl = bid % slices;
  const ReqDev rq = b.reqs[r];
  if (rq.item_begin >= b.item_hi || rq.item_begin + rq.n_items <= b.item_lo) return;
  const int item_lanes = (int)blockDim.x / op_split;
  const int per = ((rq.n_items + slices - 1) / slices + item_lanes - 1) / item_lanes * item_lanes;
  const int slice_lo = sl * per, slice_hi = min(rq.n_items, slice_lo + per);
  if (sl > 0 && slice_lo >= rq.n_items) return;
  for (int e = threadIdx.x; e < prog.n_prep; e += blockDim.x) s_po[e] = b.prep_out[(size_t)r * prog.n_prep + e];
  if (rt_doubles) {
    const uint4 *src = (const uint4 *)rt_src;
    uint4 *dst = (uint4 *)(smem + thr_at);
    for (uint32_t i = threadIdx.x; i < rt_doubles / 2; i += blockDim.x) dst[i] = src[i];
  }
  __syncthreads();
  PrepScratch sc{s_vals, vals_cap, s_int, 0ull, {0, 0, 0, 0, 0, 0}};
#ifdef MRK_PHASE_CLOCKS
  sc.clk = clock64();
#endif
  prepass_request(st, prog, b, r, rq, s_tab, (uint32_t)rq.arena_begin, s_po, sc);
  const int og = (int)threadIdx.x / item_lanes, il = (int)threadIdx.x % item_lanes;
  for (int base = slice_lo; base < slice_hi; base += item_lanes) {
    const int i = base + il;
    const int gi0 = rq.item_begin + i;
    const bool active = i < slice_hi && gi0 >= b.item_lo && gi0 < b.item_hi;
    if (!__any(active)) continue;
    const int gi = active ? gi0 : rq.item_begin;
    assemble_item<SPLIT>(st, prog, b, gi, r, rq, s_tab, (uint32_t)rq.arena_begin, s_po, make_sink(gi, r, active, s_thr, s_thr_all), og, op_split);
  }
  MRK_PHASE(sc.clk, sc.acc[5]);
#ifdef MRK_PHASE_CLOCKS
  if (threadIdx.x == 0) {
    for (int i = 0; i < 6; ++i) atomicAdd(&mrk_phase_clocks[i], sc.acc[i]);
    atomicAdd(&mrk_phase_clocks[6], 1ull);
  }
#endif
}


template <bool F64, typename QS = QsDyn, typename Prog>
__device__ __forceinline__ void assemble_cells_body(const StoreDev &st, const Prog &prog, const BatchDev &b, const QsDev &q, uint16_t *cells,
                                                    uint32_t lds_entries) {
  __shared__ __align__(16) double s_thr[ASM_THREADS / 64][2 * QS_LDS_THR];
  extern __shared__ __align__(16) unsigned long long s_tab_copy[];
  const int wg_lo = b.item_lo + (int)blockIdx.x * ASM_THREADS;
  if (wg_lo >= b.item_hi) return;
#ifdef MRK_PHASE_CLOCKS
  unsigned long long clk_t = clock64(), clk_acc[2] = {0, 0};
#endif
// ... 74 lines not shown
          __syncthreads();
          have_req = r_lo;
        }
        tab_sub = a0;
      }
    }
    const int gi0 = wg_lo + (int)threadIdx.x;
    const bool active = gi0 < b.item_hi;
    MRK_PHASE(clk_t, clk_acc[0]);
    if (__any(active)) {
      const int gi = active ? gi0 : b.item_hi - 1;
      const int r = (int)b.item_req[gi];
      const ReqDev rq = b.reqs[r];
      CellSinkRT<F64, QS> sink{q, cells + (size_t)(gi / QS_TILE_ROWS) * QS::n_views * QS_TILE_ROWS + (gi % QS_TILE_ROWS), &b.status[r], s_thr, active};
      if (in_lds) assemble_item(st, prog, b, gi, r, rq, s_tab_copy, tab_sub, &b.prep_out[(size_t)r * prog.n_prep], sink);
      else assemble_item(st, prog, b, gi, r, rq, b.arena, 0u, &b.prep_out[(size_t)r * prog.n_prep], sink);
    }
    MRK_PHASE(clk_t, clk_acc[1]);
  }
#ifdef MRK_PHASE_CLOCKS
  if (threadIdx.x == 0) {
    atomicAdd(&mrk_phase_clocks[0], clk_acc[0]);
    atomicAdd(&mrk_phase_clocks[5], clk_acc[1]);
    atomicAdd(&mrk_phase_clocks[6], 1ull);
  }
#endif
}

template <bool SPLIT = false, typename Prog>
__device__ __forceinline__ void rank_fused_matrix_body(const StoreDev &st, const Prog &prog, const BatchDev &b, uint32_t tab_entries, int vals_cap, int mode = 1) {
  rank_fused_body<SPLIT>(st, prog, b, tab_entries, vals_cap, 0u, mode,
                  [&](int gi, int, bool active, qs_lds_double *, qs_lds_double *) { return MatrixSink{b.matrix + (size_t)gi * prog.dim, active}; });
}

template <bool SPLIT = false, typename Prog>
__device__ __forceinline__ void rank_values_body(const StoreDev &st, const Prog &prog, const BatchDev &b, uint32_t tab_entries, int vals_cap,
                                                 int mode, const ValuesOut &out) {
  extern __shared__ __align__(16) uint8_t smem_base[];
  const int r = (int)blockIdx.x;
  int32_t *s_status = (int32_t *)smem_base;
  if (threadIdx.x == 0) *s_status = 0;
  BatchDev bl = b;
  bl.status = s_status - r;
  __syncthreads();
  rank_fused_body<SPLIT>(st, prog, bl, tab_entries, vals_cap, 0u, mode & 255,
                         [&](int gi, int, bool active, qs_lds_double *, qs_lds_double *) { return MatrixSink{out.matrix + (size_t)gi * prog.dim, active}; }, 16);
  __syncthreads();
  if (threadIdx.x == 0) {
    out.status[r] = *s_status;
    out.status[out.n_req_pad + r] = out.load_status ? out.load_status[r] : 0;
  }
}

template <bool F64, bool SPLIT = false, typename QS = QsDyn, typename Prog>
__device__ __forceinline__ void rank_fused_cells_body(const StoreDev &st, const Prog &prog, const BatchDev &b, uint32_t tab_entries,
                                                      int vals_cap, const QsDev &q, uint16_t *cells, int mode = 1) {
  if constexpr (qs_fused_rt<QS, SPLIT>()) {
    rank_fused_body<SPLIT>(st, prog, b, tab_entries, vals_cap, qs_thr_cap<QS>(q), mode, [&](int gi, int r, bool active, qs_lds_double *, qs_lds_double *s_all) {
      return CellSinkRT<F64, QS, !SPLIT>{q, cells + (size_t)(gi / QS_TILE_ROWS) * QS::n_views * QS_TILE_ROWS + (gi % QS_TILE_ROWS), &b.status[r], s_all, active};
    }, 0u, q.thr_rt, QS::rt_total);
  } else {
    rank_fused_body<SPLIT>(st, prog, b, tab_entries, vals_cap, qs_thr_cap<QS>(q), mode, [&](int gi, int r, bool active, qs_lds_double *s_thr, qs_lds_double *) {
      return CellSink<F64, QS>{q, cells + (size_t)(gi / QS_TILE_ROWS) * qs_n_views<QS>(q) * QS_TILE_ROWS + (gi % QS_TILE_ROWS), &b.status[r], s_thr, active};
    });
  }
}

template <bool F64, typename QS = QsDyn, typename Prog>
__device__ __forceinline__ void rank_one_body(const StoreDev &st, const Prog &prog, const BatchDev &b, uint32_t tab_entries, int vals_cap,
                                              const QsDev &q, const QsForestDev &f, int mode, const OneOut &out, int blk = -1) {
  extern __shared__ __align__(16) uint8_t smem_base[];
  const int tid = threadIdx.x, nthr = blockDim.x;
  const int r = blk < 0 ? (int)blockIdx.x : blk;
  const ReqDev rq = b.reqs[r];
  const uint32_t slab_bytes = (uint32_t)qs_n_views<QS>(q) * (QS_TILE_ROWS * 2);
  for (uint32_t i = tid; i < slab_bytes / 4 + 4; i += nthr) ((uint32_t *)smem_base)[i] = 0u;
  int32_t *s_status = (int32_t *)(smem_base + slab_bytes);
  BatchDev bl = b;
  bl.status = s_status - r;
  __syncthreads();
  if constexpr (qs_fused_rt<QS, true>()) {
    rank_fused_body<true>(st, prog, bl, tab_entries, vals_cap, qs_thr_cap<QS>(q), mode & 255, [&](int gi, int rr, bool active, qs_lds_double *, qs_lds_double *s_all) {
      return CellSinkRT<F64, QS, false>{q, (uint16_t *)smem_base + (gi - rq.item_begin), &bl.status[rr], s_all, active};
    }, slab_bytes + 16, q.thr_rt, QS::rt_total, r);
  } else {
    rank_fused_body<true>(st, prog, bl, tab_entries, vals_cap, qs_thr_cap<QS>(q), mode & 255, [&](int gi, int rr, bool active, qs_lds_double *s_thr, qs_lds_double *) {
      return CellSink<F64, QS>{q, (uint16_t *)smem_base + (gi - rq.item_begin), &bl.status[rr], s_thr, active, false};
    }, slab_bytes + 16, nullptr, 0, r);
  }
  constexpr int TREE_LEAF_BYTES = QS_LEAVES * (F64 ? 8 : 4);
  const int nw = nthr >> 6;
  uint8_t *s_leaf = smem_base + slab_bytes + 16;
  uint8_t *s_idx = s_leaf + 8 * nw * TREE_LEAF_BYTES;
  unsigned long long *s_key = (unsigned long long *)(s_idx + 8 * nw * QS_TILE_ROWS);
  const double score = qs_score_tile_split<F64>(smem_base, s_leaf, s_idx, f, nw);
  const int n = rq.n_items;
  if (tid < n) {
    out.scores[rq.item_begin + tid] = score;
    s_key[tid] = sort_key(score);
  }
  __syncthreads();
  if (tid < n) {
    const unsigned long long mine = s_key[tid];
    int before = 0;
    for (int j = 0; j < n; ++j) {
      const unsigned long long kj = s_key[j];
      before += (kj < mine || (kj == mine && j < tid)) ? 1 : 0;
    }
    out.order[rq.item_begin + before] = tid;
  }
  if (tid == 0) {
    out.status[r] = *s_status;
    out.status[out.n_req_pad + r] = out.load_status ? out.load_status[r] : 0;
  }
}
// ... 255 lines not shown
```

metarank_amd/csrc/store.hpp:

```cpp
#pragma once
#include <algorithm>
#include <cstdint>
#include <climits>
#include <cstring>
#include <memory>
#include <queue>
#include <stdexcept>
#include <string>
#include <string_view>
#include <unordered_map>
#include <vector>

#include "device_types.hpp"
#include "runtime.hpp"

namespace mrk {


enum ColKind : uint8_t { COL_SCALAR = 0, COL_COUNTER = 1, COL_PERIODIC = 2, COL_BOUNDED_LIST = 3 };


struct Column {
  std::string name;
  ColKind kind = COL_SCALAR;
  int periods = 0;
  int tag_index = 0;
  int val_off = 0;
  std::string link_field;
  bool expect_list = false;
  bool sorted_lists = false;
  int64_t period_ms = 0;
  std::vector<int32_t> offsets;
  int ring_off = -1;
  int ring_w = 0;
  int64_t list_count = INT64_MAX;
  int64_t list_duration_ms = INT64_MAX;
  uint32_t max_len = 0;
  uint32_t distinct = 0;
  std::vector<uint64_t> seen_tokens;
  void note_token(uint32_t tok) {
    const size_t w = tok >> 6;
    if (w >= seen_tokens.size()) seen_tokens.resize(std::max(w + 1, seen_tokens.size() * 2), 0);
    const uint64_t bit = 1ull << (tok & 63);
    distinct += (seen_tokens[w] & bit) ? 0u : 1u;
    seen_tokens[w] |= bit;
  }
};

constexpr int RING_MAX_RANGES = 16;
struct RingColDev {
  uint32_t ring_off, w, val_off, tag_index;
  int64_t period_ms;
  int32_t n_ranges;
  int32_t offsets[RING_MAX_RANGES];
  int32_t pad;
};
struct IncGroup { uint32_t slot, col, begin, end; };
struct IncUpdate { int64_t bucket, inc; };
constexpr unsigned long long RING_EMPTY = 0x8080808080808080ull;

struct SlotMap {
  typedef IdEntry Entry;
  std::vector<Entry> table;
  std::string ids;
  size_t n = 0;
  bool mirrored = false;
  bool regrown = false;
  std::vector<uint32_t> touched;
  static uint64_t hash(const char *s, size_t len) {
    uint64_t h = 0x9e3779b97f4a7c15ull ^ (len * 0xff51afd7ed558ccdull);
    size_t i = 0;
    for (; i + 8 <= len; i += 8) {
      uint64_t w;
      memcpy(&w, s + i, 8);
      h = (h ^ w) * 0x9fb21c651e98df25ull;
      h ^= h >> 29;
    }
    uint64_t w = 0;
    memcpy(&w, s + i, len - i);
    h = (h ^ w) * 0x9fb21c651e98df25ull;
    h ^= h >> 32;
    h *= 0xff51afd7ed558ccdull;
    h ^= h >> 29;
    return h ? h : 1;
  }
  static constexpr uint32_t NONE = 0xffffffffu;
  void prefetch(uint64_t h) const {
    if (!table.empty()) __builtin_prefetch(&table[(size_t)h & (table.size() - 1)]);
  }
  uint32_t find_hashed(uint64_t h, const char *s, size_t len) const {
    if (table.empty()) return NONE;
    const size_t mask = table.size() - 1;
    for (size_t i = (size_t)h & mask;; i = (i + 1) & mask) {
// ... 222 lines not shown
```

metarank_amd/csrc/table_device.hpp:

```cpp
#ifndef MRK_TABLE_DEVICE_HPP
#define MRK_TABLE_DEVICE_HPP

namespace mrk {

namespace {

constexpr unsigned long long TABLE_WALKED = 1ull << 63;
#ifndef MRK_TABLE_WALKED
#define MRK_TABLE_WALKED 1
#endif
__device__ __forceinline__ uint32_t tok_home(uint32_t tok, uint32_t span) { return __umulhi(tok * 2654435761u, span); }

__device__ __forceinline__ bool wave_any(bool p) { return __builtin_amdgcn_ballot_w64(p) != 0ull; }

#ifndef MRK_PROBE_W
#define MRK_PROBE_W 4
#endif
constexpr int PROBE_W = MRK_PROBE_W;

static_assert(PROBE_W == 2 || PROBE_W == 4, "bucketed tables: 2 or 4 entries per bucket");

__device__ __forceinline__ bool table_add_from(unsigned long long *tab, uint32_t nb, uint32_t tok, bool open, uint32_t bkt, uint32_t seen) {
  const unsigned long long fresh = (unsigned long long)tok | (1ull << 32);
  bool full = false;
// ... 10 lines not shown
      if (key == tok || key == 0u) { stop = (uint32_t)k; at_key = key == tok; }
    }
    const bool here = open && stop < (uint32_t)PROBE_W;
    unsigned long long *at = bp + (stop < (uint32_t)PROBE_W ? stop : 0u);
    if (here && at_key) atomicAdd(at, 1ull << 32);
    unsigned long long prev = ~0ull;
    if (here && !at_key) prev = atomicCAS(at, 0ull, fresh);
    const bool took = here && !at_key && prev == 0ull;
    const bool same = here && !at_key && (uint32_t)prev == tok;
    if (same) atomicAdd(at, 1ull << 32);
    const bool done = here && (at_key || took || same);
    const bool next = open && !here;
    if (MRK_TABLE_WALKED && next && !(e[0] & TABLE_WALKED)) atomicOr(bp, TABLE_WALKED);
    seen += next ? 1u : 0u;
    bkt = next ? (bkt + 1u == nb ? 0u : bkt + 1u) : bkt;
    full = full || (open && !done && seen >= nb);
    open = open && !done && seen < nb;
  }
  return !full;
}

__device__ __forceinline__ uint32_t table_get_from(const unsigned long long *tab, uint32_t nb, uint32_t tok, bool open, uint32_t bkt, uint32_t seen,
                                                   uint32_t res) {
  for (; wave_any(open); ++seen) {
    const unsigned long long *bp = tab + bkt * (uint32_t)PROBE_W;
    unsigned long long e[PROBE_W];
#pragma unroll
    for (int k = 0; k < PROBE_W; ++k) e[k] = bp[k];
    uint32_t r2 = 0u, lo = 0xffffffffu;
#pragma unroll
    for (int k = 0; k < PROBE_W; ++k) {
      const uint32_t key = (uint32_t)e[k];
      r2 = key == tok ? (uint32_t)(e[k] >> 32) & 0x7fffffffu : r2;
      lo = min(lo, key);
    }
    res = open ? r2 : res;
    open = open && r2 == 0u && lo != 0u && (!MRK_TABLE_WALKED || (e[0] & TABLE_WALKED) != 0ull) && seen + 1u < nb;
    bkt = bkt + 1u == nb ? 0u : bkt + 1u;
  }
  return res;
}

__device__ __forceinline__ bool table_add(unsigned long long *tab, uint32_t cap, uint32_t tok, bool want) {
  const uint32_t nb = cap / (uint32_t)PROBE_W;
  return table_add_from(tab, nb, tok, want, tok_home(tok, nb), 0u);
}

__device__ __forceinline__ uint32_t table_get(const unsigned long long *tab, uint32_t cap, uint32_t tok_in, bool want) {
  const uint32_t tok = want ? tok_in : 0u;
  const uint32_t nb = cap / (uint32_t)PROBE_W;
  return table_get_from(tab, nb, tok, want, tok_home(tok, nb), 0u, 0u);
}

#ifndef MRK_TOK_BATCH
#define MRK_TOK_BATCH 8
#endif
constexpr int TOK_BATCH = MRK_TOK_BATCH;

__device__ __forceinline__ uint32_t table_add_list(const uint32_t *toks, unsigned long long *tab, uint32_t cap, uint32_t len) {
  uint32_t failed = 0;
  for (uint32_t j0 = 0; wave_any(j0 < len); j0 += TOK_BATCH) {
    uint32_t tk[TOK_BATCH];
#pragma unroll
    for (int t = 0; t < TOK_BATCH; ++t) tk[t] = j0 + t < len ? toks[j0 + t] : 0u;
#pragma unroll
    for (int t = 0; t < TOK_BATCH; ++t) {
      if (!wave_any(j0 + t < len)) break;
      failed += table_add(tab, cap, tk[t], j0 + t < len) ? 0u : 1u;
    }
  }
  return failed;
}

template <int N>
__device__ __forceinline__ double table_sum_tokens(const unsigned long long *tab, uint32_t cap, const uint32_t (&tk)[N], uint32_t len, double cnt) {
#pragma unroll
  for (int t = 0; t < N; ++t) {
    if (!wave_any((uint32_t)t < len)) break;
    cnt = cnt + (double)table_get(tab, cap, tk[t], (uint32_t)t < len);
  }
  return cnt;
}

__device__ __forceinline__ double table_sum_list(const uint32_t *toks, const unsigned long long *tab, uint32_t cap, uint32_t len,
                                                 double cnt = 0.0) {
  for (uint32_t j0 = 0; wave_any(j0 < len); j0 += TOK_BATCH) {
    uint32_t tk[TOK_BATCH];
#pragma unroll
    for (int t = 0; t < TOK_BATCH; ++t) tk[t] = j0 + t < len ? toks[j0 + t] : 0u;
    cnt = table_sum_tokens<TOK_BATCH>(tab, cap, tk, len > j0 ? len - j0 : 0u, cnt);
  }
  return cnt;
}

}

}

#endif
```

metarank_amd/ranker.py:

```python
from __future__ import annotations

import ctypes as C
import json

import numpy as np

from . import _native as N
from .booster import Context, HipBooster, default_context
from .request import Request, RequestSet, request_array


def _strs(vals):
    bs = [v.encode() for v in vals]
    return (C.c_char_p * max(len(bs), 1))(*bs), bs


class Batch:

    def __init__(self, ranker: "HipRanker", model_name: str | None = None, events=None):
        self.ranker = ranker
        self._h = C.c_void_p()
        self.requests, self.n_req, self.total_items, self.dim, self.offsets = [], 0, 0, 0, np.zeros(1, dtype=np.int64)
        if events is None:
            N.check(N.lib().mrk_batch_create(ranker.ctx.handle, C.byref(self._h)))
# ... 61 lines not shown
        c = N.lib().mrk_batch_shard_chunk(self._h, shard_count)
        if c < 0:
            N.check(c)
        return c

    def run_sharded(self, booster: HipBooster | None):
        N.check(N.lib().mrk_batch_run_sharded(self._h, booster.handle if booster is not None else None))

    def allgather_scores(self):
        N.check(N.lib().mrk_batch_allgather_scores(self._h))

    def gather_scores(self) -> int:
        p = C.c_void_p()
        N.check(N.lib().mrk_batch_gather_scores(self._h, C.byref(p)))
        return p.value

    def sort(self):
        N.check(N.lib().mrk_batch_sort(self._h))

    def sync(self):
        N.check(N.lib().mrk_batch_sync(self._h))

    @property
    def stream(self):
        return N.lib().mrk_batch_stream(self._h)

    def device_outputs(self, matrix: bool = False):
        s, o, m = C.c_void_p(), C.c_void_p(), C.c_void_p()
        N.check(N.lib().mrk_batch_device_outputs(self._h, C.byref(s), C.byref(o), C.byref(m) if matrix else None))
        return s.value, o.value, (m.value if matrix else None)

    def fetch(self, matrix: bool = False):
        scores = np.empty(self.total_items, dtype=np.float64)
        order = np.empty(self.total_items, dtype=np.int32)
        mat = np.empty((self.total_items, self.dim), dtype=np.float64) if matrix else None
        N.check(N.lib().mrk_batch_fetch(self._h, scores.ctypes.data_as(C.c_void_p), order.ctypes.data_as(C.c_void_p),
                                        mat.ctypes.data_as(C.c_void_p) if matrix else None))
        return scores, order, mat

    def status(self) -> np.ndarray:
        st = np.zeros(max(self.n_req, 1), dtype=np.int32)
        N.check(N.lib().mrk_batch_status(self._h, st.ctypes.data_as(C.c_void_p)))
        return st[:self.n_req]

    def tables(self):
        fn = N.lib().mrk_debug_batch_tables
        fn.restype, fn.argtypes = C.c_int, [C.c_void_p, C.POINTER(C.c_int64), C.c_void_p, C.c_int64]
        out = (C.c_int64 * 3)()
        N.check(fn(self._h, out, None, 0))
        caps = np.zeros((int(out[1]), int(out[2])), dtype=np.uint32)
        N.check(fn(self._h, out, caps.ctypes.data_as(C.c_void_p), caps.size))
        return int(out[0]), caps

    def close(self):
        if self._h:
            N.lib().mrk_batch_free(self._h)
            self._h = C.c_void_p()

    def __del__(self):
        try:
            self.close()
        except Exception:
            pass


class HipRanker:
    def __init__(self, config: dict, ctx: Context | None = None):
        self.ctx = ctx or default_context()
        self._own_ctx = False
        if getattr(self.ctx, "_configured", False):
            self.ctx = Context(self.ctx.device)
            self._own_ctx = True
        self.config = config
        blob = json.dumps({"features": config["features"], "models": config.get("models", {})}).encode()
        N.check(N.lib().mrk_config_load_json(self.ctx.handle, blob, len(blob)))
        self.ctx._configured = True

    def _k(self, key): return key.encode()
    def put_double(self, key, v): N.check(N.lib().mrk_store_put_double(self.ctx.handle, self._k(key), float(v)))
    def put_bool(self, key, v): N.check(N.lib().mrk_store_put_bool(self.ctx.handle, self._k(key), 1 if v else 0))
    def put_string(self, key, v): N.check(N.lib().mrk_store_put_string(self.ctx.handle, self._k(key), v.encode()))

    def put_string_list(self, key, v):
        arr, _keep = _strs(v)
        N.check(N.lib().mrk_store_put_string_list(self.ctx.handle, self._k(key), arr, len(v)))

    def put_double_list(self, key, v):
        a = np.ascontiguousarray(v, dtype=np.float64)
        N.check(N.lib().mrk_store_put_double_list(self.ctx.handle, self._k(key), a.ctypes.data_as(C.c_void_p), len(a)))

    def put_counter(self, key, v): N.check(N.lib().mrk_store_put_counter(self.ctx.handle, self._k(key), int(v)))

    def put_periodic(self, key, v):
        a = np.ascontiguousarray(v, dtype=np.int64)
        N.check(N.lib().mrk_store_put_periodic(self.ctx.handle, self._k(key), a.ctypes.data_as(C.c_void_p), len(a)))

    def put_bounded_list(self, key, v):
        arr, _keep = _strs(v)
        N.check(N.lib().mrk_store_put_bounded_list(self.ctx.handle, self._k(key), arr, len(v)))

    def increment_periodic(self, key, ts_ms, inc=1):
        N.check(N.lib().mrk_store_increment_periodic(self.ctx.handle, self._k(key), int(ts_ms), int(inc)))

    def increment(self, key, inc=1):
        N.check(N.lib().mrk_store_increment(self.ctx.handle, self._k(key), int(inc)))

    def append(self, key, value, ts_ms):
        N.check(N.lib().mrk_store_append(self.ctx.handle, self._k(key), str(value).encode(), int(ts_ms)))

    def put_binary(self, blob: bytes, now_ms: int | None = None) -> int:
        n = C.c_int(0)
        if now_ms is None:
            N.check(N.lib().mrk_store_put_binary(self.ctx.handle, blob, len(blob), C.byref(n)))
        else:
            N.check(N.lib().mrk_store_put_binary_at(self.ctx.handle, blob, len(blob), now_ms, C.byref(n)))
        return n.value
# ... 160 lines not shown
```

Before: 1.166 billion.

## Use compact 32-bit LDS hash tables in fused rank kernel when tokens fit

```diff
diff --git a/metarank_amd/__init__.py b/metarank_amd/__init__.py
--- a/metarank_amd/__init__.py
+++ b/metarank_amd/__init__.py
@@ -1,7 +1,7 @@
 from ._native import MrkError, build, lib, reload_switches
 from .booster import LIGHTGBM, XGBOOST, Context, HipBooster, default_context
 from .index import HipIndex
-from .ranker import Batch, HipRanker, Server
+from .ranker import Batch, HipRanker, Server, debug_fused_lds
 from .request import Request, RequestSet
 from .trending import HipTrending, TrendingBuilder
 from .als import AlsBuilder
diff --git a/metarank_amd/_native.py b/metarank_amd/_native.py
--- a/metarank_amd/_native.py
+++ b/metarank_amd/_native.py
@@ -29,7 +29,7 @@
     return [os.path.join(CSRC, f) for f in SOURCES + extra]
 
 
-JIT_HEADERS = ["device_types.hpp", "rank.hpp", "qs_device.hpp", "sort_device.hpp", "table_device.hpp", "walk_device.hpp", "wave_device.hpp", "rank_device.hpp"]
+JIT_HEADERS = ["device_types.hpp", "rank.hpp", "qs_device.hpp", "sort_device.hpp", "table_device.hpp", "table32_device.hpp", "walk_device.hpp", "wave_device.hpp", "rank_device.hpp"]
 
 
 def embed_jit_sources() -> str:
diff --git a/metarank_amd/csrc/capi_rank.cpp b/metarank_amd/csrc/capi_rank.cpp
--- a/metarank_amd/csrc/capi_rank.cpp
+++ b/metarank_amd/csrc/capi_rank.cpp
@@ -36,9 +36,10 @@
                         int *d_status, const uint32_t *d_row_req);
 void launch_assemble_cells(mrk_ctx *ctx, const StoreDev &st, const ProgramDev &prog, const BatchDev &b, const QsDev &q,
                            uint16_t *cells, bool f64, void *jit_fn, uint32_t max_req_entries, void *jit_rt_fn = nullptr, uint32_t thr_total = 0);
-void launch_rank_fused(mrk_ctx *ctx, const StoreDev &st, const ProgramDev &prog, const BatchDev &b, uint32_t tab_entries,
-                       int vals_cap, int threads, int op_split, int slices, const QsDev *q, uint16_t *cells, bool f64, void *jit_fn, size_t rt_bytes = 0);
-size_t fused_lds_bytes(uint32_t tab_entries, int vals_cap, int threads, uint32_t thr_cap, size_t rt_bytes, bool split);
+size_t launch_rank_fused(mrk_ctx *ctx, const StoreDev &st, const ProgramDev &prog, const BatchDev &b, uint32_t tab_entries,
+                         int vals_cap, int threads, int op_split, int slices, const QsDev *q, uint16_t *cells, bool f64, void *jit_fn, size_t rt_bytes = 0,
+                         int entry_bytes = 8, bool split_kernel = false);
+size_t fused_lds_bytes(uint32_t tab_entries, int vals_cap, int threads, uint32_t thr_cap, size_t rt_bytes, bool split, int entry_bytes = 8);
 size_t fused_rt_max_bytes();
 int fused_max_prep();
 QsDev qs_device_view(const mrk_model *m);
@@ -115,6 +116,9 @@
   int fused_vals = 1, fused_threads = 64;
   int fused_slices = 1;
   int fused_split = 1;
+  int ran_entry_bytes = 0, ran_kernel = 0;
+  size_t ran_lds = 0, ran_rt_bytes = 0;
+  uint32_t ran_thr_cap = 0;
   bool want_matrix = false;
   bool matrix_valid = false;
   bool values = false;
@@ -429,12 +433,13 @@
                            b.fused_slices == 1 && b.hb.max_items <= QS_TILE_ROWS && b.view.n_overrides == 0 && b.big.empty() && b.fused_threads <= 256 &&
                            rank_fused_score_lds_bytes(b.fused_entries, b.fused_vals, b.fused_threads, qs_device_view(model).thr_cap, qs_device_view(model).n_views, f64, (size_t)qs_device_view(model).rt_doubles * 8) <= 64 * 1024;
   const QsSignature *sig = cells && sw.thr_stage ? &model->qs_sig : nullptr;
+  const bool plain = b.fused_split == 1 && b.fused_slices == 1, compact = b.hb.compact_tables;
   void *jit_fn = one_walk ? jit_one_walk_function(*b.prog, f64)
                  : !cells ? (b.fused_ok && model && b.fused_split == 1 && b.fused_slices == 1 ? jit_matrix_function(*b.prog) : nullptr)
                         : one ? jit_one_function(*b.prog, f64, sig)
                         : fused_score ? jit_fused_score_function(*b.prog, f64, sig)
                         : !b.fused_ok ? jit_items_function(*b.prog, f64, sig)
-                        : b.fused_split > 1 || b.fused_slices > 1 ? jit_split_function(*b.prog, f64, sig) : jit_rank_function(*b.prog, f64, sig);
+                        : !plain || !compact ? jit_split_function(*b.prog, f64, sig) : jit_rank_function(*b.prog, f64, sig);
   void *jit_rt_fn = cells && !one && !fused_score && !b.fused_ok ? jit_items_rt_function(*b.prog, f64, sig) : nullptr;
   void *jit_prep_fn = cells && !one && !fused_score && !b.fused_ok && b.prog->prep.size() && sw.jit_prepass ? jit_prepass_function(*b.prog) : nullptr;
   LaunchOn on(ctx, b.s());
@@ -443,6 +448,8 @@
   b.fetch_enqueued = false;
   b.direct_out = false;
   b.values_ran = b.values_direct = false;
+  b.ran_entry_bytes = b.ran_kernel = 0;
+  b.ran_lds = 0;
   if (one || one_walk) {
     b.h_out.reserve(b.out_bytes);
     uint8_t *h = b.h_out.as<uint8_t>();
@@ -478,8 +485,12 @@
     if (hi % QS_TILE_ROWS && tile_bytes)
       MRK_HIP(hipMemsetAsync(b.d_cells.as<uint8_t>() + (size_t)(hi / QS_TILE_ROWS) * tile_bytes, 0, tile_bytes, b.s()));
     if (b.fused_ok) {
-      launch_rank_fused(ctx, st, pd, b.view, b.fused_entries, b.fused_vals, b.fused_threads, b.fused_split, b.fused_slices, &q, b.d_cells.as<uint16_t>(), f64, jit_fn,
-                        sig && sig->ok ? (size_t)sig->rt_total * 8 : 0);
+      b.ran_kernel = !jit_fn ? 0 : plain && compact ? 1 : 2;
+      b.ran_entry_bytes = b.ran_kernel == 1 ? 4 : 8;
+      b.ran_rt_bytes = sig && sig->ok ? (size_t)sig->rt_total * 8 : 0;
+      b.ran_thr_cap = q.thr_cap;
+      b.ran_lds = launch_rank_fused(ctx, st, pd, b.view, b.fused_entries, b.fused_vals, b.fused_threads, b.fused_split, b.fused_slices, &q, b.d_cells.as<uint16_t>(), f64, jit_fn,
+                                    b.ran_rt_bytes, b.ran_entry_bytes, b.ran_kernel == 2);
     } else {
       launch_prepass(ctx, st, pd, b.view, b.fused_entries, jit_prep_fn);
       launch_assemble_cells(ctx, st, pd, b.view, q, b.d_cells.as<uint16_t>(), f64, jit_fn, b.fused_entries, jit_rt_fn, jit_rt_fn ? model->qs_sig.rt_total : 0u);
@@ -890,6 +901,25 @@
     if (!caps) return;
     if (n_caps < (int64_t)n || b->hb.prep_out.size() < n) throw StatusError(MRK_ERR_INVALID_ARG, "caps is too short");
     for (size_t i = 0; i < n; ++i) caps[i] = b->hb.prep_out[i].tab_cap;
+  });
+}
+
+int mrk_debug_batch_launch(mrk_batch *b, int64_t *out10) {
+  return guard([&] {
+    if (!b || !out10) throw StatusError(MRK_ERR_INVALID_ARG, "null argument");
+    std::lock_guard<std::mutex> lk(b->bmu);
+    out10[0] = b->ran_entry_bytes; out10[1] = (int64_t)b->ran_lds; out10[2] = b->ran_kernel; out10[3] = b->hb.compact_tables ? 1 : 0;
+    out10[4] = b->fused_entries; out10[5] = b->fused_vals; out10[6] = b->fused_threads; out10[7] = b->ran_thr_cap; out10[8] = (int64_t)b->ran_rt_bytes;
+    out10[9] = b->fused_split > 1 || b->fused_slices > 1 || b->ran_kernel == 2 ? 1 : 0;
+  });
+}
+
+int mrk_debug_fused_lds(int64_t insertions, int64_t max_token, int64_t tab_entries, int64_t vals_cap, int64_t threads, int64_t thr_cap, int64_t rt_bytes,
+                        int split, int entry_bytes, int64_t *out2) {
+  return guard([&] {
+    if (!out2 || insertions < 0 || max_token < 0 || (entry_bytes != 4 && entry_bytes != 8)) throw StatusError(MRK_ERR_INVALID_ARG, "bad argument");
+    out2[0] = compact_table_ok((uint64_t)insertions, (uint32_t)std::min<int64_t>(max_token, 0xffffffffll)) ? 1 : 0;
+    out2[1] = (int64_t)fused_lds_bytes((uint32_t)tab_entries, (int)vals_cap, (int)threads, (uint32_t)thr_cap, (size_t)rt_bytes, split != 0, entry_bytes);
   });
 }
 
diff --git a/metarank_amd/csrc/features.cpp b/metarank_amd/csrc/features.cpp
--- a/metarank_amd/csrc/features.cpp
+++ b/metarank_amd/csrc/features.cpp
@@ -971,6 +971,7 @@
   hb.irf.clear();
   hb.overrides.clear();
   hb.arena_entries = hb.max_req_entries = 0;
+  hb.compact_tables = true;
   hb.max_doubles = hb.max_items = hb.total_items = 0;
   std::vector<int> begins((size_t)n_req + 1, 0);
   for (int r = 0; r < n_req; ++r) {
@@ -1071,7 +1072,8 @@
   const Table &item_table = store.tables[SC_ITEM];
   auto col_max_len = [&](ColRef c) -> uint64_t { return c.tag >= 0 && c.tag < (int)item_table.cols.size() ? item_table.cols[(size_t)c.tag].max_len : 0u; };
   auto vocab_bound = [&](ColRef c) -> uint64_t { return c.tag >= 0 && c.tag < (int)item_table.cols.size() ? 2ull * item_table.cols[(size_t)c.tag].distinct : 0u; };
-  struct Worker { std::vector<Override> overrides; int max_items = 0, max_doubles = 0; std::vector<double> enc; };
+  auto col_max_token = [&](ColRef c) -> uint32_t { return c.tag >= 0 && c.tag < (int)item_table.cols.size() ? item_table.cols[(size_t)c.tag].max_token : 0u; };
+  struct Worker { std::vector<Override> overrides; int max_items = 0, max_doubles = 0; std::vector<double> enc; bool compact = true; };
   std::vector<Worker> workers((size_t)std::max(1, n_workers));
   std::vector<uint64_t> req_entries((size_t)n_req, 0);
   auto resolve_one = [&](int r, Worker &wk, int item_workers) {
@@ -1244,6 +1246,7 @@
           }
           PrepOut &po = hb.prep_out[(size_t)r * prog.prep.size() + ho.prep_base + fi];
           const uint32_t cap = table_capacity(std::min(count, vocab_bound(pe.item_col)), load_pct);
+          wk.compact = wk.compact && compact_table_ok(count, col_max_token(pe.item_col));
           po.tab_off = (uint32_t)arena;
           po.tab_cap = cap;
           arena += cap;
@@ -1297,6 +1300,7 @@
         }
         wk.max_doubles = std::max(wk.max_doubles, doubles);
         const uint32_t cap = table_capacity(std::min(tokens, vocab_bound(pe.item_col)), load_pct);
+        wk.compact = wk.compact && compact_table_ok(tokens, col_max_token(pe.item_col));
         po.tab_off = (uint32_t)arena;
         po.tab_cap = cap;
         arena += cap;
@@ -1399,6 +1403,7 @@
     hb.overrides.insert(hb.overrides.end(), wk.overrides.begin(), wk.overrides.end());
     hb.max_items = std::max(hb.max_items, wk.max_items);
     hb.max_doubles = std::max(hb.max_doubles, wk.max_doubles);
+    hb.compact_tables = hb.compact_tables && wk.compact;
   }
   for (const CrossValue &c : cross_values)
     if (c.v == c.v) hb.overrides.push_back({(uint32_t)(hb.reqs[c.req].item_begin + c.item), (uint32_t)c.dst, c.v});
diff --git a/metarank_amd/csrc/features.hpp b/metarank_amd/csrc/features.hpp
--- a/metarank_amd/csrc/features.hpp
+++ b/metarank_amd/csrc/features.hpp
@@ -110,12 +110,17 @@
   std::vector<PrepOut> prep_out;
   uint64_t arena_entries = 0;
   uint64_t max_req_entries = 0;
+  bool compact_tables = true;
   int max_doubles = 0;
   int max_items = 0;
   int total_items = 0;
   bool device_ids = false;
 };
 
+constexpr uint32_t COMPACT_MAX_TOKEN = (1u << 20) - 1u;
+constexpr uint64_t COMPACT_MAX_COUNT = 2047;
+inline bool compact_table_ok(uint64_t insertions, uint32_t max_token) { return insertions <= COMPACT_MAX_COUNT && max_token <= COMPACT_MAX_TOKEN; }
+
 void resolve_requests(const Program &prog, Store &store, const mrk_request *reqs, int n_req, const mrk_item_ids *ids, HostBatch &out);
 
 }
diff --git a/metarank_amd/csrc/jit.cpp b/metarank_amd/csrc/jit.cpp
--- a/metarank_amd/csrc/jit.cpp
+++ b/metarank_amd/csrc/jit.cpp
@@ -94,14 +94,16 @@
     qs = "mrk::JitQs";
   }
   s += "}  // namespace\n}  // namespace mrk\n\n";
-  std::string attr;
+  std::string attr, attr_rank;
   {
-    const int w = switches().jit_waves >= 1 && switches().jit_waves <= 8 ? switches().jit_waves : 4;
+    const bool forced = switches().jit_waves >= 1 && switches().jit_waves <= 8;
+    const int w = forced ? switches().jit_waves : 4, wr = forced ? switches().jit_waves : 5;
     attr = " __attribute__((amdgpu_waves_per_eu(" + std::to_string(w) + ", " + std::to_string(w) + ")))";
+    attr_rank = " __attribute__((amdgpu_waves_per_eu(" + std::to_string(wr) + ", " + std::to_string(wr) + ")))";
   }
   const std::string b64 = f64 ? "true" : "false";
   if (kernel == JIT_ALL || kernel == JIT_RANK)
-    s += "extern \"C\" __global__ void __launch_bounds__(256)" + attr + "\nmrk_jit_rank_cells"
+    s += "extern \"C\" __global__ void __launch_bounds__(256)" + attr_rank + "\nmrk_jit_rank_cells"
          "(mrk::StoreDev st, mrk::BatchDev b, uint32_t tab_entries, int vals_cap, mrk::QsDev q, uint16_t *cells, int mode) {\n"
          "  mrk::rank_fused_cells_body<" + b64 + ", false, " + qs + ">(st, mrk::JitProg{}, b, tab_entries, vals_cap, q, cells, mode);\n}\n";
   if (kernel == JIT_ALL || kernel == JIT_SPLIT)
diff --git a/metarank_amd/csrc/rank.hip b/metarank_amd/csrc/rank.hip
--- a/metarank_amd/csrc/rank.hip
+++ b/metarank_amd/csrc/rank.hip
@@ -297,20 +297,21 @@
   launch_override_cells(ctx, b, q, cells, f64);
 }
 
-size_t fused_lds_bytes(uint32_t tab_entries, int vals_cap, int threads, uint32_t thr_cap, size_t rt_bytes, bool split) {
+size_t fused_lds_bytes(uint32_t tab_entries, int vals_cap, int threads, uint32_t thr_cap, size_t rt_bytes, bool split, int entry_bytes = 8) {
   const size_t staging = (size_t)((threads + 63) / 64) * 2 * thr_cap * 8;
-  return (size_t)tab_entries * 8 + (size_t)vals_cap * 8 + FUSED_MAX_PREP * sizeof(PrepOut) + PREP_INTS * sizeof(int) +
+  return (((size_t)tab_entries * (size_t)entry_bytes + 7) & ~(size_t)7) + (size_t)vals_cap * 8 + FUSED_MAX_PREP * sizeof(PrepOut) + PREP_INTS * sizeof(int) +
          16 + std::max(staging, rt_bytes <= (split ? FUSED_RT_MAX_BYTES_SPLIT : FUSED_RT_MAX_BYTES) ? rt_bytes : 0);
 }
 size_t fused_rt_max_bytes() { return FUSED_RT_MAX_BYTES_SPLIT; }
 int fused_max_prep() { return FUSED_MAX_PREP; }
 
-void launch_rank_fused(mrk_ctx *ctx, const StoreDev &st, const ProgramDev &prog, const BatchDev &b, uint32_t tab_entries,
-                       int vals_cap, int threads, int op_split, int slices, const QsDev *q, uint16_t *cells, bool f64, void *jit_fn, size_t rt_bytes) {
-  if (b.n_req <= 0) return;
+size_t launch_rank_fused(mrk_ctx *ctx, const StoreDev &st, const ProgramDev &prog, const BatchDev &b, uint32_t tab_entries,
+                         int vals_cap, int threads, int op_split, int slices, const QsDev *q, uint16_t *cells, bool f64, void *jit_fn, size_t rt_bytes,
+                         int entry_bytes, bool split_kernel) {
+  if (b.n_req <= 0) return 0;
   int mode = (op_split > 1 ? op_split : 1) | ((slices > 1 ? slices : 1) << 8);
   const unsigned grid = (unsigned)b.n_req * (unsigned)(slices > 1 ? slices : 1);
-  size_t lds = fused_lds_bytes(tab_entries, vals_cap, threads, q ? q->thr_cap : 0u, q && cells ? rt_bytes : 0, op_split > 1 || slices > 1);
+  size_t lds = fused_lds_bytes(tab_entries, vals_cap, threads, q ? q->thr_cap : 0u, q && cells ? rt_bytes : 0, op_split > 1 || slices > 1 || split_kernel, entry_bytes);
   if (switches().fused_lds_min > 0) lds = std::max(lds, (size_t)switches().fused_lds_min);
   {
     ScopedKernelTimer timer(ctx, "assemble");
@@ -342,6 +343,7 @@
   } else {
     launch_override_cells(ctx, b, *q, cells, f64);
   }
+  return lds;
 }
 
 size_t rank_values_lds_bytes(uint32_t tab_entries, int vals_cap, int threads) { return 16 + fused_lds_bytes(tab_entries, vals_cap, threads, 0u, 0, true); }
diff --git a/metarank_amd/csrc/rank_device.hpp b/metarank_amd/csrc/rank_device.hpp
--- a/metarank_amd/csrc/rank_device.hpp
+++ b/metarank_amd/csrc/rank_device.hpp
@@ -5,6 +5,7 @@
 #include "rank.hpp"
 #include "sort_device.hpp"
 #include "table_device.hpp"
+#include "table32_device.hpp"
 #include "walk_device.hpp"
 #include "wave_device.hpp"
 
@@ -199,9 +200,9 @@
   return ok;
 }
 
-template <typename Prog>
+template <typename Prog, typename T>
 __device__ __forceinline__ void prepass_interacted_with(const StoreDev &st, const Prog &prog, const BatchDev &b, int r, const ReqDev &rq,
-                                                        unsigned long long *tab_base, uint32_t tab_sub, PrepOut *po_out, int lane_id, int n_lanes) {
+                                                        T *tab_base, uint32_t tab_sub, PrepOut *po_out, int lane_id, int n_lanes) {
   const int n_prep = prog.n_prep;
   for (int e0 = 0; e0 < n_prep;) {
     const PrepEntry pe0 = prog.prep[e0];
@@ -213,7 +214,7 @@
       ++n;
     }
     ColRef col[PREP_GROUP];
-    unsigned long long *tab[PREP_GROUP];
+    T *tab[PREP_GROUP];
     uint32_t cap[PREP_GROUP];
 #pragma unroll
     for (int u = 0; u < PREP_GROUP; ++u) {
@@ -250,9 +251,9 @@
 
 }
 
-template <typename Prog>
+template <typename Prog, typename T>
 __device__ __forceinline__ void prepass_diversity_wave(const StoreDev &st, const Prog &prog, const BatchDev &b, int r, const ReqDev &rq,
-                                                       unsigned long long *tab_base, uint32_t tab_sub, PrepOut *po_out, const PrepScratch &sc) {
+                                                       T *tab_base, uint32_t tab_sub, PrepOut *po_out, const PrepScratch &sc) {
   const int lane = threadIdx.x & 63;
   const int n_prep = prog.n_prep;
   int *s_first = sc.first();
@@ -271,7 +272,7 @@
       ++n;
     }
     ColRef col[DIV_GROUP];
-    unsigned long long *tab[DIV_GROUP];
+    T *tab[DIV_GROUP];
     uint32_t cap[DIV_GROUP];
     int top[DIV_GROUP];
 #pragma unroll
@@ -352,7 +353,7 @@
             const bool take = cand[u] && running[u] + excl < top[u];
             const bool one = take && c[u].tag == TAG_STRING;
             const uint32_t tlen = take && !one ? c[u].hi() : 0u;
-            uint32_t failed = table_add(tab[u], cap[u], c[u].lo(), one) ? 0u : 1u;
+            uint32_t failed = TableOps<T>::add(tab[u], cap[u], c[u].lo(), one) ? 0u : 1u;
             failed += table_add_list(list_tokens(st, irec, c[u].lo()), tab[u], cap[u], tlen);
             if (failed) atomicOr(&b.status[r], ST_TABLE_FULL);
             if (take) atomicAdd(&s_tokens[u], one ? 1 : (int)tlen);
@@ -409,9 +410,9 @@
 #endif
 }
 
-template <typename Prog>
+template <typename Prog, typename T>
 __device__ __forceinline__ void prepass_request(const StoreDev &st, const Prog &prog, const BatchDev &b, int r, const ReqDev &rq,
-                                unsigned long long *tab_base, uint32_t tab_sub, PrepOut *po_out, const PrepScratch &sc) {
+                                T *tab_base, uint32_t tab_sub, PrepOut *po_out, const PrepScratch &sc) {
   const int tid = threadIdx.x;
   const int nthr = blockDim.x;
   const int n_prep = prog.n_prep;
@@ -426,7 +427,7 @@
       lo = min(lo, o);
       hi = max(hi, o + po_out[e].tab_cap);
     }
-    for (uint32_t i = lo + tid; i < hi; i += nthr) tab_base[i] = 0ull;
+    for (uint32_t i = lo + tid; i < hi; i += nthr) tab_base[i] = (T)0;
     for (int e = tid; e < n_prep; e += nthr) s_first[e] = 0x7fffffff;
   }
   __syncthreads();
@@ -456,7 +457,7 @@
       ++n;
     }
     ColRef col[PREP_GROUP];
-    unsigned long long *tab[PREP_GROUP];
+    T *tab[PREP_GROUP];
     uint32_t cap[PREP_GROUP];
 #pragma unroll
     for (int u = 0; u < PREP_GROUP; ++u) {
@@ -502,7 +503,7 @@
       ++n;
     }
     ColRef col[PREP_GROUP];
-    unsigned long long *tab[PREP_GROUP];
+    T *tab[PREP_GROUP];
     uint32_t cap[PREP_GROUP];
     int top[PREP_GROUP];
 #pragma unroll
@@ -584,7 +585,7 @@
             const bool take = cand[u] && running[u] + excl[u] < top[u];
             const bool one = take && c[u].tag == TAG_STRING;
             const uint32_t tlen = take && !one ? c[u].hi() : 0u;
-            uint32_t failed = table_add(tab[u], cap[u], c[u].lo(), one) ? 0u : 1u;
+            uint32_t failed = TableOps<T>::add(tab[u], cap[u], c[u].lo(), one) ? 0u : 1u;
             failed += table_add_list(list_tokens(st, irec, c[u].lo()), tab[u], cap[u], tlen);
             if (failed) atomicOr(&b.status[r], ST_TABLE_FULL);
             if (take) atomicAdd(&s_tokens[u], one ? 1 : (int)tlen);
@@ -1132,9 +1133,9 @@
   }
 }
 
-template <bool SPLIT, typename Prog, typename Sink, typename IR>
+template <bool SPLIT, typename Prog, typename Sink, typename IR, typename T>
 __device__ __forceinline__ void assemble_item_rec(const StoreDev &st, const Prog &prog, const BatchDev &b, int gi, int r,
-                                                  const ReqDev &rq, const unsigned long long *tab_base, uint32_t tab_sub,
+                                                  const ReqDev &rq, const T *tab_base, uint32_t tab_sub,
                                                   const PrepOut *pos, const Sink &sink, int islot, const IR &ir, int og, int G_arg) {
   const int G = SPLIT ? G_arg : 1;
   const uint8_t *irec = ir.p;
@@ -1416,7 +1417,7 @@
           for (int u = 0; u < IW_BATCH; ++u) {
             if (f0 + u >= op.dim) break;
             const PrepOut po = pos[op.i1 + f0 + u];
-            const unsigned long long *tab = tab_base + (po.tab_off - tab_sub);
+            const T *tab = tab_base + (po.tab_off - tab_sub);
             const uint32_t len = fc[u].tag == TAG_STRING_LIST ? fc[u].hi() : 0u;
             double cnt = table_sum_tokens<IW_TOK>(tab, po.tab_cap, tk[u], len, 0.0);
             if (wave_any(len > (uint32_t)IW_TOK))
@@ -1435,9 +1436,9 @@
         } else if (po.mode == DIV_DOUBLE) {
           if (c.tag == TAG_DOUBLE) v = c.f64() - po.scalar;
         } else {
-          const unsigned long long *tab = tab_base + (po.tab_off - tab_sub);
+          const T *tab = tab_base + (po.tab_off - tab_sub);
           const bool one = c.tag == TAG_STRING, list = c.tag == TAG_STRING_LIST;
-          const double w1 = 0.0 + (double)table_get(tab, po.tab_cap, c.lo(), one);
+          const double w1 = 0.0 + (double)TableOps<T>::get(tab, po.tab_cap, c.lo(), one);
           const uint32_t len = list ? c.hi() : 0u;
           uint32_t dtk[TOK_BATCH];
 #pragma unroll
@@ -1580,9 +1581,9 @@
 template <typename P> __device__ __forceinline__ constexpr int prog_item_pieces(...) { return 0; }
 constexpr int REC_MAX_PIECES = 24;
 
-template <bool SPLIT = false, typename Prog, typename Sink>
+template <bool SPLIT = false, typename Prog, typename Sink, typename T>
 __device__ __forceinline__ void assemble_item(const StoreDev &st, const Prog &prog, const BatchDev &b, int gi, int r,
-                                              const ReqDev &rq, const unsigned long long *tab_base, uint32_t tab_sub,
+                                              const ReqDev &rq, const T *tab_base, uint32_t tab_sub,
                                               const PrepOut *pos, const Sink &sink, int og = 0, int G = 1) {
   const int islot = sink.active ? b.item_slot[gi] : -1;
   const uint8_t *irec = record(st, SC_ITEM, islot);
@@ -1597,7 +1598,7 @@
 }
 
 
-template <bool SPLIT, typename Prog, typename SinkMaker>
+template <bool SPLIT, typename T = unsigned long long, typename Prog, typename SinkMaker>
 __device__ __forceinline__ void rank_fused_body(const StoreDev &st, const Prog &prog, const BatchDev &b, uint32_t tab_entries,
                                                 int vals_cap, uint32_t thr_cap, int mode, const SinkMaker &make_sink, uint32_t lds_skip = 0,
                                                 const double *rt_src = nullptr, uint32_t rt_doubles = 0, int blk = -1) {
@@ -1605,9 +1606,10 @@
   const int slices = SPLIT ? (((mode >> 8) & 255) > 1 ? ((mode >> 8) & 255) : 1) : 1;
   extern __shared__ __align__(16) uint8_t smem_base[];
   uint8_t *smem = smem_base + lds_skip;
-  unsigned long long *s_tab = (unsigned long long *)smem;
-  double *s_vals = (double *)(smem + (size_t)tab_entries * 8);
-  PrepOut *s_po = (PrepOut *)(smem + (size_t)tab_entries * 8 + (size_t)vals_cap * 8);
+  T *s_tab = (T *)smem;
+  const size_t tab_bytes = sizeof(T) == 8 ? (size_t)tab_entries * 8 : ((size_t)tab_entries * sizeof(T) + 7) & ~(size_t)7;
+  double *s_vals = (double *)(smem + tab_bytes);
+  PrepOut *s_po = (PrepOut *)(smem + tab_bytes + (size_t)vals_cap * 8);
   int *s_int = (int *)(s_po + FUSED_MAX_PREP);
   const size_t thr_at = ((size_t)((uint8_t *)(s_int + PREP_INTS) - smem) + 15) & ~(size_t)15;
   qs_lds_double *s_thr_all = (qs_lds_double *)(smem + thr_at);
@@ -1788,15 +1790,17 @@
   }
 }
 
-template <bool F64, bool SPLIT = false, typename QS = QsDyn, typename Prog>
+template <bool SPLIT> struct FusedCellsEntry { typedef unsigned long long type; };
+template <> struct FusedCellsEntry<false> { typedef uint32_t type; };
+template <bool F64, bool SPLIT = false, typename QS = QsDyn, typename T = typename FusedCellsEntry<SPLIT>::type, typename Prog>
 __device__ __forceinline__ void rank_fused_cells_body(const StoreDev &st, const Prog &prog, const BatchDev &b, uint32_t tab_entries,
                                                       int vals_cap, const QsDev &q, uint16_t *cells, int mode = 1) {
   if constexpr (qs_fused_rt<QS, SPLIT>()) {
-    rank_fused_body<SPLIT>(st, prog, b, tab_entries, vals_cap, qs_thr_cap<QS>(q), mode, [&](int gi, int r, bool active, qs_lds_double *, qs_lds_double *s_all) {
+    rank_fused_body<SPLIT, T>(st, prog, b, tab_entries, vals_cap, qs_thr_cap<QS>(q), mode, [&](int gi, int r, bool active, qs_lds_double *, qs_lds_double *s_all) {
       return CellSinkRT<F64, QS, !SPLIT>{q, cells + (size_t)(gi / QS_TILE_ROWS) * QS::n_views * QS_TILE_ROWS + (gi % QS_TILE_ROWS), &b.status[r], s_all, active};
     }, 0u, q.thr_rt, QS::rt_total);
   } else {
-    rank_fused_body<SPLIT>(st, prog, b, tab_entries, vals_cap, qs_thr_cap<QS>(q), mode, [&](int gi, int r, bool active, qs_lds_double *s_thr, qs_lds_double *) {
+    rank_fused_body<SPLIT, T>(st, prog, b, tab_entries, vals_cap, qs_thr_cap<QS>(q), mode, [&](int gi, int r, bool active, qs_lds_double *s_thr, qs_lds_double *) {
       return CellSink<F64, QS>{q, cells + (size_t)(gi / QS_TILE_ROWS) * qs_n_views<QS>(q) * QS_TILE_ROWS + (gi % QS_TILE_ROWS), &b.status[r], s_thr, active};
     });
   }
diff --git a/metarank_amd/csrc/store.hpp b/metarank_amd/csrc/store.hpp
--- a/metarank_amd/csrc/store.hpp
+++ b/metarank_amd/csrc/store.hpp
@@ -37,8 +37,10 @@
   int64_t list_duration_ms = INT64_MAX;
   uint32_t max_len = 0;
   uint32_t distinct = 0;
+  uint32_t max_token = 0;
   std::vector<uint64_t> seen_tokens;
   void note_token(uint32_t tok) {
+    max_token = std::max(max_token, tok);
     const size_t w = tok >> 6;
     if (w >= seen_tokens.size()) seen_tokens.resize(std::max(w + 1, seen_tokens.size() * 2), 0);
     const uint64_t bit = 1ull << (tok & 63);
diff --git a/metarank_amd/csrc/table32_device.hpp b/metarank_amd/csrc/table32_device.hpp
--- /dev/null
+++ b/metarank_amd/csrc/table32_device.hpp
@@ -0,0 +1,98 @@
+#ifndef MRK_TABLE32_DEVICE_HPP
+#define MRK_TABLE32_DEVICE_HPP
+
+namespace mrk {
+
+namespace {
+
+constexpr uint32_t T32_KEY_SHIFT = 12;
+constexpr uint32_t T32_WALKED = 1u << 11;
+constexpr uint32_t T32_COUNT_MASK = T32_WALKED - 1u;
+constexpr uint32_t T32_MAX_TOKEN = (1u << (32 - T32_KEY_SHIFT)) - 1u;
+
+struct __attribute__((aligned(8))) T32Pair { uint32_t x, y; };
+
+__device__ __forceinline__ void table32_bucket(const uint32_t *bp, uint32_t (&e)[PROBE_W]) {
+  const T32Pair *hp = (const T32Pair *)bp;
+  T32Pair h[PROBE_W / 2];
+#pragma unroll
+  for (int k = 0; k < PROBE_W / 2; ++k) h[k] = hp[k];
+#pragma unroll
+  for (int k = 0; k < PROBE_W / 2; ++k) { e[2 * k] = h[k].x; e[2 * k + 1] = h[k].y; }
+}
+
+__device__ __forceinline__ bool table32_add_from(uint32_t *tab, uint32_t nb, uint32_t tok, bool open, uint32_t bkt, uint32_t seen) {
+  const uint32_t fresh = (tok << T32_KEY_SHIFT) | 1u;
+  bool full = false;
+  while (wave_any(open)) {
+    uint32_t *bp = tab + bkt * (uint32_t)PROBE_W;
+    uint32_t e[PROBE_W];
+    table32_bucket(bp, e);
+    uint32_t stop = PROBE_W;
+    bool at_key = false;
+#pragma unroll
+    for (int k = PROBE_W - 1; k >= 0; --k) {
+      const uint32_t key = e[k] >> T32_KEY_SHIFT;
+      if (key == tok || e[k] == 0u) { stop = (uint32_t)k; at_key = e[k] != 0u; }
+    }
+    const bool here = open && stop < (uint32_t)PROBE_W;
+    uint32_t *at = bp + (stop < (uint32_t)PROBE_W ? stop : 0u);
+    if (here && at_key) atomicAdd(at, 1u);
+    const bool tried = here && !at_key;
+    uint32_t prev = 0u;
+    if (tried) prev = atomicCAS(at, 0u, fresh);
+    const bool took = tried && prev == 0u;
+    const bool same = tried && (prev >> T32_KEY_SHIFT) == tok;
+    if (same) atomicAdd(at, 1u);
+    const bool done = here && (at_key || took || same);
+    const bool next = open && !here;
+    if (MRK_TABLE_WALKED && next && !(e[0] & T32_WALKED)) atomicOr(bp, T32_WALKED);
+    seen += next ? 1u : 0u;
+    bkt = next ? (bkt + 1u == nb ? 0u : bkt + 1u) : bkt;
+    full = full || (open && !done && seen >= nb);
+    open = open && !done && seen < nb;
+  }
+  return !full;
+}
+
+__device__ __forceinline__ uint32_t table32_get_from(const uint32_t *tab, uint32_t nb, uint32_t tok, bool open, uint32_t bkt, uint32_t seen, uint32_t res) {
+  const uint32_t tk = tok << T32_KEY_SHIFT;
+  for (; wave_any(open); ++seen) {
+    const uint32_t *bp = tab + bkt * (uint32_t)PROBE_W;
+    uint32_t e[PROBE_W];
+    table32_bucket(bp, e);
+    uint32_t hit = 0xffffffffu, lo = 0xffffffffu;
+#pragma unroll
+    for (int k = 0; k < PROBE_W; ++k) {
+      hit = min(hit, e[k] ^ tk);
+      lo = min(lo, e[k]);
+    }
+    const uint32_t r2 = hit < (1u << T32_KEY_SHIFT) ? hit & T32_COUNT_MASK : 0u;
+    res = open ? r2 : res;
+    open = open && r2 == 0u && lo != 0u && (!MRK_TABLE_WALKED || (e[0] & T32_WALKED) != 0u) && seen + 1u < nb;
+    bkt = bkt + 1u == nb ? 0u : bkt + 1u;
+  }
+  return res;
+}
+
+__device__ __forceinline__ bool table_add(uint32_t *tab, uint32_t cap, uint32_t tok, bool want) {
+  const uint32_t nb = cap / (uint32_t)PROBE_W;
+  return table32_add_from(tab, nb, tok, want, tok_home(tok, nb), 0u);
+}
+
+__device__ __forceinline__ uint32_t table_get(const uint32_t *tab, uint32_t cap, uint32_t tok_in, bool want) {
+  const uint32_t tok = want ? tok_in : 0u;
+  const uint32_t nb = cap / (uint32_t)PROBE_W;
+  return table32_get_from(tab, nb, tok, want, tok_home(tok, nb), 0u, 0u);
+}
+
+template <> struct TableOps<uint32_t> {
+  static __device__ __forceinline__ bool add(uint32_t *tab, uint32_t cap, uint32_t tok, bool want) { return table_add(tab, cap, tok, want); }
+  static __device__ __forceinline__ uint32_t get(const uint32_t *tab, uint32_t cap, uint32_t tok, bool want) { return table_get(tab, cap, tok, want); }
+};
+
+}
+
+}
+
+#endif
diff --git a/metarank_amd/csrc/table_device.hpp b/metarank_amd/csrc/table_device.hpp
--- a/metarank_amd/csrc/table_device.hpp
+++ b/metarank_amd/csrc/table_device.hpp
@@ -86,12 +86,19 @@
   return table_get_from(tab, nb, tok, want, tok_home(tok, nb), 0u, 0u);
 }
 
+template <typename T> struct TableOps;
+template <> struct TableOps<unsigned long long> {
+  static __device__ __forceinline__ bool add(unsigned long long *tab, uint32_t cap, uint32_t tok, bool want) { return table_add(tab, cap, tok, want); }
+  static __device__ __forceinline__ uint32_t get(const unsigned long long *tab, uint32_t cap, uint32_t tok, bool want) { return table_get(tab, cap, tok, want); }
+};
+
 #ifndef MRK_TOK_BATCH
 #define MRK_TOK_BATCH 8
 #endif
 constexpr int TOK_BATCH = MRK_TOK_BATCH;
 
-__device__ __forceinline__ uint32_t table_add_list(const uint32_t *toks, unsigned long long *tab, uint32_t cap, uint32_t len) {
+template <typename T>
+__device__ __forceinline__ uint32_t table_add_list(const uint32_t *toks, T *tab, uint32_t cap, uint32_t len) {
   uint32_t failed = 0;
   for (uint32_t j0 = 0; wave_any(j0 < len); j0 += TOK_BATCH) {
     uint32_t tk[TOK_BATCH];
@@ -100,23 +107,24 @@
 #pragma unroll
     for (int t = 0; t < TOK_BATCH; ++t) {
       if (!wave_any(j0 + t < len)) break;
-      failed += table_add(tab, cap, tk[t], j0 + t < len) ? 0u : 1u;
+      failed += TableOps<T>::add(tab, cap, tk[t], j0 + t < len) ? 0u : 1u;
     }
   }
   return failed;
 }
 
-template <int N>
-__device__ __forceinline__ double table_sum_tokens(const unsigned long long *tab, uint32_t cap, const uint32_t (&tk)[N], uint32_t len, double cnt) {
+template <int N, typename T>
+__device__ __forceinline__ double table_sum_tokens(const T *tab, uint32_t cap, const uint32_t (&tk)[N], uint32_t len, double cnt) {
 #pragma unroll
   for (int t = 0; t < N; ++t) {
     if (!wave_any((uint32_t)t < len)) break;
-    cnt = cnt + (double)table_get(tab, cap, tk[t], (uint32_t)t < len);
+    cnt = cnt + (double)TableOps<T>::get(tab, cap, tk[t], (uint32_t)t < len);
   }
   return cnt;
 }
 
-__device__ __forceinline__ double table_sum_list(const uint32_t *toks, const unsigned long long *tab, uint32_t cap, uint32_t len,
+template <typename T>
+__device__ __forceinline__ double table_sum_list(const uint32_t *toks, const T *tab, uint32_t cap, uint32_t len,
                                                  double cnt = 0.0) {
   for (uint32_t j0 = 0; wave_any(j0 < len); j0 += TOK_BATCH) {
     uint32_t tk[TOK_BATCH];
diff --git a/metarank_amd/ranker.py b/metarank_amd/ranker.py
--- a/metarank_amd/ranker.py
+++ b/metarank_amd/ranker.py
@@ -137,6 +137,13 @@
         N.check(fn(self._h, out, caps.ctypes.data_as(C.c_void_p), caps.size))
         return int(out[0]), caps
 
+    def launch_info(self) -> dict:
+        fn = N.lib().mrk_debug_batch_launch
+        fn.restype, fn.argtypes = C.c_int, [C.c_void_p, C.POINTER(C.c_int64)]
+        out = (C.c_int64 * 10)()
+        N.check(fn(self._h, out))
+        return dict(zip(("entry_bytes", "lds", "kernel", "qualifies", "tab_entries", "vals_cap", "threads", "thr_cap", "rt_bytes", "split"), [int(x) for x in out]))
+
     def close(self):
         if self._h:
             N.lib().mrk_batch_free(self._h)
@@ -147,6 +154,15 @@
             self.close()
         except Exception:
             pass
+
+
+def debug_fused_lds(insertions: int, max_token: int, tab_entries: int = 0, vals_cap: int = 1, threads: int = 64, thr_cap: int = 0, rt_bytes: int = 0,
+                    split: bool = False, entry_bytes: int = 8):
+    fn = N.lib().mrk_debug_fused_lds
+    fn.restype, fn.argtypes = C.c_int, [C.c_int64] * 7 + [C.c_int, C.c_int, C.POINTER(C.c_int64)]
+    out = (C.c_int64 * 2)()
+    N.check(fn(insertions, max_token, tab_entries, vals_cap, threads, thr_cap, rt_bytes, int(split), entry_bytes, out))
+    return bool(out[0]), int(out[1])
 
 
 class HipRanker:
```

Measured after the change: 1.209 billion (median of 6 runs). 1.04x the previous value.
